# rdd0582/mri_superresolution

Hardware: AMD Instinct MI355X
Metric: 2D MRI slices/sec (train fwd+bwd) 256×256 U-Net; PSNR/SSIM vs ref (higher is better)
Workload: dtype bf16; 1 GPU; UNetSuperRes base_filters=64 depth=4, 256x256 slices -> 512x512, batch=16/GPU bf16, L1+SSIM(0.4), train step fwd+bwd+Adam+SSIM metric; global_batch=16, parallelism=dp1

## Files before the change

include/mrisr.h:

```cpp
#ifndef MRISR_H
#define MRISR_H

#include <stddef.h>
#include <stdint.h>

#ifdef __cplusplus
extern "C" {
#endif

#define MRISR_OK 0
#define MRISR_E_ARG (-1)
#define MRISR_E_SHAPE (-2)
#define MRISR_E_DTYPE (-3)
#define MRISR_E_HIP (-4)
#define MRISR_E_UNSUPPORTED (-5)

#define MRISR_F32 0
#define MRISR_BF16 1
#define MRISR_F16 2

#define MRISR_SRC_RAW 0
#define MRISR_SRC_NORM 1
#define MRISR_SRC_RELU 2
#define MRISR_SP_NONE 0
#define MRISR_SP_POOL2 1
#define MRISR_SP_UP2 2
#define MRISR_COMBINE_CONCAT 0
#define MRISR_COMBINE_BLEND 1
#ifndef MRISR_STAT_SLOTS
#define MRISR_STAT_SLOTS 16
#endif
#define MRISR_SP_HEAD 3
#define MRISR_OUT_PLAIN 0
#define MRISR_OUT_PIXEL_SHUFFLE2 1

typedef struct {
    const void* ptr;
    const float* scale;
    const float* shift;
    int32_t C, H, W;
    int32_t mode;
    int32_t spatial;
    int32_t off_y, off_x;
} mrisr_src;

typedef struct {
    int32_t dtype;
    int32_t N, H, W;
    int32_t Cin, Cout;
    int32_t ksize;
    int32_t nsrc;
    int32_t combine;
    int32_t out_mode;
    int32_t groups;
    int32_t relu_out;
    mrisr_src src[2];
    const float* blend_alpha;
    const void* wpacked;
    const float* bias;
    void* out;
    double* stats;
    const void* relu_mask;
    int32_t cu_limit;
    int32_t reserved_;
    const void* wpacked_ring;
} mrisr_conv_desc;

const char* mrisr_last_error(void);
int mrisr_version(void);
int mrisr_stat_slots(void);

size_t mrisr_packed_weight_bytes(int dtype, int Cout, int Cin, int ksize);
#define MRISR_PACK_RING 256
#define MRISR_PACK_UPADJ 512
int mrisr_conv_ring_bn(int dtype, int Cout, int Cin, int ksize);
size_t mrisr_packed_weight_bytes_ring(int dtype, int Cout, int Cin, int ksize);
int mrisr_pack_weights(int dtype, const float* w, int Cout, int Cin, int ksize, int transpose_flip,
                       void* packed, void* stream);
typedef struct {
    const float* w;
    void* packed;
    int32_t Cout, Cin, ksize, transpose_flip;
} mrisr_pack_job;
int mrisr_pack_weights_batched(int dtype, const mrisr_pack_job* jobs_device, int njobs, void* stream);
int mrisr_conv_forward(const mrisr_conv_desc* d, void* stream);
int mrisr_conv_variant(const mrisr_conv_desc* d, int wgrad, char* out, size_t n);
int mrisr_conv_wgrad(const mrisr_conv_desc* d, const void* dy, float* dw, float* workspace, size_t workspace_floats,
                     void* stream);
size_t mrisr_conv_wgrad_workspace_floats(const mrisr_conv_desc* d);

size_t mrisr_packed_weight_bytes_upadj(int dtype, int Cout, int Cin, int ksize);
int mrisr_conv_upadj(const mrisr_conv_desc* d, const void* g, void* d_low, void* stream);

int mrisr_stem_forward(int dtype, const float* x, const float* w, void* out, double* stats,
                       int N, int H, int W, int Cout, int groups, void* stream);
int mrisr_stem_wgrad(int dtype, const float* x, const void* dy, float* dw,
                     int N, int H, int W, int Cout, void* stream);
int mrisr_stem_forward_multi(int dtype, const float* x, const float* w, void* out, double* stats,
                             int N, int H, int W, int Cin, int Cout, int groups, void* stream);
int mrisr_stem_wgrad_multi(int dtype, const float* x, const void* dy, float* dw,
                           int N, int H, int W, int Cin, int Cout, void* stream);

int mrisr_gn_finalize(const double* stats, const float* gamma, const float* beta, float* scale,
                      float* shift, float* meanrstd, int N, int C, int groups, double count,
                      float eps, void* stream);

int mrisr_norm_pool2(int dtype, const void* x, const float* scale, const float* shift, void* out, int N,
                     int H, int W, int C, void* stream);
int mrisr_norm_upsample2(int dtype, const void* x, const float* scale, const float* shift, void* out, int N,
                         int h, int w, int C, void* stream);
int mrisr_norm_blend(int dtype, const void* x0, const float* scale0, const float* shift0, const void* x1,
                     const float* scale1, const float* shift1, const float* alpha, void* out, int N, int H, int W,
                     int C, void* stream);
int mrisr_upsample2_stats(int dtype, const void* z_low, void* z, double* stats, int N, int h, int w, int C,
                          int groups, void* stream);
int mrisr_upsample2_adjoint(int dtype, const void* dz, void* dz_low, int N, int h, int w, int C, void* stream);

typedef struct {
    const void* da;
    int32_t C_total;
    int32_t c_off;
    int32_t H, W;
    int32_t spatial;
    int32_t off_y, off_x;
    int32_t weight_mode;
    const float* head_out;
    const float* head_w;
    float* head_part;
    float* head_dw;
    float* head_db;
} mrisr_consumer;

int mrisr_act_bwd_reduce(int dtype, const void* x, const float* scale, const float* shift,
                         const float* meanrstd, int nconsumers, const mrisr_consumer* consumers,
                         const float* blend_alpha, void* g, float* red, float* alpha_slots, int N, int H, int W,
                         int C, int groups, void* stream);
int mrisr_act_bwd_finalize(const float* red, const float* gamma, const float* meanrstd, float* dgamma,
                           float* dbeta, float* coef, int N, int C, int groups, double count,
                           const float* alpha_slots, const float* alpha, float* dalpha, float alpha_sign, void* stream);
int mrisr_act_bwd_apply(int dtype, const void* x, const void* g, const float* coef, void* dx, int N,
                        int H, int W, int C, int out_mode, float* dbias, void* stream);
typedef struct mrisr_gn_bwd_fin {
    const float* red;
    const float* gamma;
    const float* meanrstd;
    float* dgamma;
    float* dbeta;
    const float* alpha_slots;
    const float* alpha;
    float* dalpha;
    double count;
    float alpha_sign;
    int32_t groups;
} mrisr_gn_bwd_fin;
int mrisr_act_bwd_apply_fused(int dtype, const void* x, const float* scale, const float* shift, int nconsumers,
                              const mrisr_consumer* consumers, const float* blend_alpha, const float* coef,
                              const mrisr_gn_bwd_fin* fin, void* dx, int N, int H, int W, int C, void* stream);
int mrisr_act_bwd_onepass_slots(void);
int mrisr_act_bwd_onepass_barrier_words(void);
int mrisr_act_bwd_onepass_ok(int dtype, int nconsumers, const mrisr_consumer* consumers, int N, int H, int W, int C);
int mrisr_act_bwd_onepass(int dtype, const void* x, const float* scale, const float* shift, const float* meanrstd,
                          int nconsumers, const mrisr_consumer* consumers, float* red, uint32_t* arrive,
                          const mrisr_gn_bwd_fin* fin, void* dx, int N, int H, int W, int C, void* stream);
int mrisr_act_bwd_apply_fused_unshuffle(int dtype, const void* x, const float* scale, const float* shift,
                                        const mrisr_consumer* consumer, const float* blend_alpha,
                                        const mrisr_gn_bwd_fin* fin, void* dx, float* dbias, int N, int H, int W, int C,
                                        void* stream);
typedef struct mrisr_blend_branch {
    const void* x;
    const float* scale;
    const float* shift;
    const float* meanrstd;
    float* red;
    float* alpha_slots;
    int32_t weight_mode;
    int32_t reserved_;
} mrisr_blend_branch;
int mrisr_act_bwd_blend_ok(int dtype, int N, int H, int W, int C);
int mrisr_act_bwd_blend_reduce(int dtype, const void* da, const mrisr_blend_branch* ps, const mrisr_blend_branch* bil,
                               const float* blend_alpha, int N, int H, int W, int C, int groups, void* stream);
int mrisr_act_bwd_blend_apply(int dtype, const void* da, const mrisr_blend_branch* ps, const mrisr_blend_branch* bil,
                              const float* blend_alpha, const mrisr_gn_bwd_fin* fin_ps, const mrisr_gn_bwd_fin* fin_bil,
                              void* dx_ps, void* dx_bil, float* dbias, int N, int H, int W, int C, void* stream);
int mrisr_channel_sum(int dtype, const void* x, float* out, size_t npix, int C, void* stream);

int mrisr_head_forward(int dtype, const void* x, const float* scale, const float* shift,
                       const float* w, const float* b, float* out, int N, int H, int W, int C,
                       void* stream);
int mrisr_head_backward(int dtype, const void* x, const float* scale, const float* shift,
                        const float* w, const float* out, const float* dout, void* da, float* dw,
                        float* db, int N, int H, int W, int C, void* stream);
int mrisr_head_forward_multi(int dtype, const void* x, const float* scale, const float* shift,
                             const float* w, const float* b, float* out, int N, int H, int W, int C,
                             int K, void* stream);
int mrisr_head_backward_multi(int dtype, const void* x, const float* scale, const float* shift,
                              const float* w, const float* out, const float* dout, void* da,
                              float* dw, float* db, int N, int H, int W, int C, int K, void* stream);

int mrisr_ssim_l1_forward(const float* a, const float* b, double* sums, float* coef, int N, int H,
                          int W, float val_range, float sigma, void* stream);
int mrisr_ssim_l1_backward(const float* a, const float* b, const float* coef, const double* sums,
                           const float* gscale, float l1_w, float ssim_w, float* da, int N, int H,
                           int W, float sigma, void* stream);
int mrisr_ssim_l1_forward_win(const float* a, const float* b, double* sums, float* coef, int N, int H, int W,
                              float val_range, float sigma, int window_size, void* stream);
int mrisr_ssim_l1_backward_win(const float* a, const float* b, const float* coef, const double* sums,
                               const float* gscale, float l1_w, float ssim_w, float* da, int N, int H, int W,
                               float sigma, int window_size, void* stream);

int mrisr_loss_finalize(const double* sums, int N, int H, int W, float l1_w, float ssim_w, float* out,
                        void* stream);

int mrisr_image_metrics(const float* a, const float* b, double* sums, int N, int H, int W, float val_range, float sigma,
                        int window_size, void* stream);
int mrisr_metrics_finalize(const double* sums, int N, int H, int W, float val_range, double* out, void* stream);

int mrisr_vgg_input_channels(void);
int mrisr_vgg_input_forward(int dtype, const float* x, void* out, size_t npix, void* stream);
int mrisr_vgg_input_backward(int dtype, const void* dx3, const float* gscale, float scale, float* dimg,
                             size_t npix, void* stream);
int mrisr_maxpool2_forward(int dtype, const void* x, void* out, int N, int H, int W, int C, void* stream);
int mrisr_maxpool2_backward(int dtype, const void* x, const void* dy, void* dx, int N, int H, int W, int C,
                            int relu_gate, void* stream);
int mrisr_feature_loss(int dtype, const void* a, const void* b, size_t n, int kind, double* sum16, float* out,
                       void* da, int relu_gate, void* stream);

int mrisr_adam_step(float* p, const float* g, float* m, float* v, size_t n, float lr, float beta1,
                    float beta2, float eps, float weight_decay, int step, float grad_scale,
                    void* stream);
int mrisr_adam_step_amp(float* p, const float* g, float* m, float* v, size_t n, float lr, float beta1, float beta2,
                        float eps, float weight_decay, int* step_device, float grad_mul,
                        const float* loss_scale_device, const float* found_inf_device, void* stream);

int mrisr_u8_histogram(const uint8_t* img, size_t pixels_per_image, int batch, unsigned* hist, void* stream);
int mrisr_u8_percentile_normalise(const uint8_t* img, const unsigned* hist, size_t pixels_per_image, int batch,
                                  double q_lo, double q_hi, float* out, float* lohi, void* stream);
int mrisr_f32_to_u8(const float* x, uint8_t* out, size_t n, void* stream);

#define MRISR_UP2_BILINEAR 0
#define MRISR_UP2_BICUBIC 1
#define MRISR_UP2_SHARP_BILINEAR 2
int mrisr_u8_upscale2(const uint8_t* in, uint8_t* out_u8, float* out_f32, int batch, int h, int w, int method, void* stream);
int mrisr_u8_to_unit_f32(const uint8_t* img, float* out, size_t n, void* stream);

typedef struct {
    float cos_a, sin_a;
    int32_t rotate;
    int32_t flip;
    int32_t fill;
    float brightness;
} mrisr_aug_geo;
typedef struct {
    float contrast;
    int32_t mean;
    float noise_sigma;
    uint32_t seed;
} mrisr_aug_photo;
int mrisr_augment_geo_u8(const uint8_t* in, uint8_t* out, int batch, int H, int W, const mrisr_aug_geo* params_device,
                         const double* mean_device, void* stream);
int mrisr_augment_finish_u8(const uint8_t* in, float* out, int batch, size_t pixels_per_image,
                            const mrisr_aug_photo* params_device, const double* mean_device, void* stream);

int mrisr_lowfield_dirichlet(int n, double crop_factor, float* re, float* im);
size_t mrisr_lowfield_workspace_bytes(int batch, int H, int W);
int mrisr_lowfield_simulate(const uint8_t* high, int batch, int H, int W, double crop_factor, const float* row_re,
                            const float* row_im, const float* col_re, const float* col_im, float sigma,
                            const float* noise_re, const float* noise_im, const unsigned long long* seeds_device,
                            void* workspace, uint8_t* out_u8, float* out_f32, void* stream);

int mrisr_lowfield_dirichlet_any(int n, double crop_factor, float* re, float* im);
int mrisr_lowfield_simulate_f32(const float* high, int batch, int H, int W, double crop_factor, const float* row_re,
                                const float* row_im, const float* col_re, const float* col_im, float sigma,
                                const float* noise_re, const float* noise_im, const unsigned long long* seeds_device,
                                void* workspace, float* out_f32, void* stream);

#define MRISR_WINDOW_F32 0
#define MRISR_WINDOW_I16 1
size_t mrisr_f32_percentile_workspace_bytes(int batch);
int mrisr_f32_percentile_bounds(const float* x, size_t pixels_per_image, int batch, double q_lo, double q_hi, float* lohi,
                                void* workspace, void* stream);
int mrisr_f32_window_normalise(const float* x, const float* lohi, size_t pixels_per_image, int batch, float* out, void* stream);
int mrisr_f32_window_restore(const float* y, const float* lohi, size_t pixels_per_image, int batch, int out_dtype, void* out,
                             void* stream);

#define MRISR_RESAMPLE_LINEAR 1
#define MRISR_RESAMPLE_CUBIC 2
#define MRISR_RESAMPLE_AREA 3
#define MRISR_RESAMPLE_LANCZOS4 4
int mrisr_resample_taps(int method, int src, int dst, int max_taps, int* ntaps, short* index, float* weight);
int mrisr_f32_resample_letterbox(const float* in, int batch, int H, int W, const short* y_index, const float* y_weight,
                                 int y_taps, int new_h, const short* x_index, const float* x_weight, int x_taps, int new_w,
                                 int out_h, int out_w, int y_off, int x_off, float pad_value, int clip, float* out_f32,
                                 uint8_t* out_u8, void* stream);

#define MRISR_VOLBLEND_SET 0
#define MRISR_VOLBLEND_ADD 1
#define MRISR_VOLBLEND_FINISH 2
int mrisr_f32_volume_up2_blend(const float* plane, int axis, int X, int Y, int Z, float* acc, int mode, int count, int out_dtype,
                               void* out, void* stream);

int mrisr_f32_volume_down2(const float* src, int X, int Y, int Z, int axes_mask, float* dst, void* stream);
int mrisr_f32_volume_up2(const float* src, int X, int Y, int Z, int axes_mask, int method, float* dst, void* stream);
int mrisr_f32_volume_metrics(const float* a, const float* b, int X, int Y, int Z, float val_range, float sigma, int window_size,
                             double* sums, void* stream);
int mrisr_volume_metrics_finalize(const double* sums, int X, int Y, int Z, float val_range, double* out, void* stream);
int mrisr_f32_volume_metrics_masked(const float* a, const float* b, const uint8_t* mask, int X, int Y, int Z, float val_range,
                                    float sigma, int window_size, double* sums7, void* stream);
int mrisr_volume_metrics_finalize_masked(const double* sums7, int X, int Y, int Z, float val_range, double* out11, void* stream);

size_t mrisr_f32_volume_otsu_workspace_bytes(void);
int mrisr_f32_volume_otsu_mask(const float* vol, int X, int Y, int Z, uint8_t* mask_out, double* stats, void* workspace,
                               void* stream);
#define MRISR_MORPH_DILATE 0
#define MRISR_MORPH_ERODE 1
int mrisr_u8_volume_morph(const uint8_t* src, int X, int Y, int Z, int radius, int op, uint8_t* dst, uint8_t* tmp, void* stream);

int mrisr_u8_volume_label(const uint8_t* mask, int X, int Y, int Z, int connectivity, int plane_axis, int invert, int32_t* labels,
                          void* stream);
size_t mrisr_u8_volume_label_workspace_bytes(int X, int Y, int Z);
int mrisr_u8_volume_keep_largest(const uint8_t* mask, int X, int Y, int Z, int connectivity, uint8_t* dst, double* stats3,
                                 void* workspace, void* stream);
int mrisr_u8_volume_fill_holes(const uint8_t* mask, int X, int Y, int Z, int plane_axis, uint8_t* dst, double* stats1, void* workspace,
                               void* stream);

#ifdef __cplusplus
}
#endif
#endif
```

mri_superresolution_amd/_lib.py:

```python
from __future__ import annotations

import ctypes as C
import os

from .tuning import TUNING

_HERE = os.path.dirname(os.path.abspath(__file__))
LIB_PATH = TUNING.lib_path or os.path.join(_HERE, "libmrisr.so")

F32, BF16, F16 = 0, 1, 2
SRC_RAW, SRC_NORM, SRC_RELU = 0, 1, 2
SP_NONE, SP_POOL2, SP_UP2, SP_HEAD = 0, 1, 2, 3
COMBINE_CONCAT, COMBINE_BLEND = 0, 1
OUT_PLAIN, OUT_PIXEL_SHUFFLE2 = 0, 1
UP2_BILINEAR, UP2_BICUBIC, UP2_SHARP_BILINEAR = 0, 1, 2
WINDOW_F32, WINDOW_I16 = 0, 1
VOLBLEND_SET, VOLBLEND_ADD, VOLBLEND_FINISH = 0, 1, 2
MORPH_DILATE, MORPH_ERODE = 0, 1
RESAMPLE_LINEAR, RESAMPLE_CUBIC, RESAMPLE_AREA, RESAMPLE_LANCZOS4 = 1, 2, 3, 4
PACK_RING = 256
PACK_UPADJ = 512
STAT_SLOTS = 16

_vp, _fp, _dp, _i, _f, _d, _sz = C.c_void_p, C.c_void_p, C.c_void_p, C.c_int, C.c_float, C.c_double, C.c_size_t


class Src(C.Structure):
    _fields_ = [("ptr", _vp), ("scale", _fp), ("shift", _fp), ("C", C.c_int32), ("H", C.c_int32),
                ("W", C.c_int32), ("mode", C.c_int32), ("spatial", C.c_int32), ("off_y", C.c_int32),
                ("off_x", C.c_int32)]


class ConvDesc(C.Structure):
    _fields_ = [("dtype", C.c_int32), ("N", C.c_int32), ("H", C.c_int32), ("W", C.c_int32),
                ("Cin", C.c_int32), ("Cout", C.c_int32), ("ksize", C.c_int32), ("nsrc", C.c_int32),
                ("combine", C.c_int32), ("out_mode", C.c_int32), ("groups", C.c_int32),
                ("relu_out", C.c_int32), ("src", Src * 2), ("blend_alpha", _fp), ("wpacked", _vp),
                ("bias", _fp), ("out", _vp), ("stats", _dp), ("relu_mask", _vp), ("cu_limit", C.c_int32),
                ("reserved_", C.c_int32), ("wpacked_ring", _vp)]


class PackJob(C.Structure):
    _fields_ = [("w", _fp), ("packed", _vp), ("Cout", C.c_int32), ("Cin", C.c_int32), ("ksize", C.c_int32),
                ("transpose_flip", C.c_int32)]


class AugGeo(C.Structure):
    _fields_ = [("cos_a", C.c_float), ("sin_a", C.c_float), ("rotate", C.c_int32), ("flip", C.c_int32),
                ("fill", C.c_int32), ("brightness", C.c_float)]


class AugPhoto(C.Structure):
    _fields_ = [("contrast", C.c_float), ("mean", C.c_int32), ("noise_sigma", C.c_float), ("seed", C.c_uint32)]


class GnBwdFin(C.Structure):
    _fields_ = [("red", _fp), ("gamma", _fp), ("meanrstd", _fp), ("dgamma", _fp), ("dbeta", _fp),
                ("alpha_slots", _fp), ("alpha", _fp), ("dalpha", _fp), ("count", C.c_double),
                ("alpha_sign", C.c_float), ("groups", C.c_int32)]


class BlendBranch(C.Structure):
    _fields_ = [("x", _vp), ("scale", _fp), ("shift", _fp), ("meanrstd", _fp), ("red", _fp), ("alpha_slots", _fp),
                ("weight_mode", C.c_int32), ("reserved_", C.c_int32)]


class Consumer(C.Structure):
    _fields_ = [("da", _vp), ("C_total", C.c_int32), ("c_off", C.c_int32), ("H", C.c_int32),
                ("W", C.c_int32), ("spatial", C.c_int32), ("off_y", C.c_int32), ("off_x", C.c_int32),
                ("weight_mode", C.c_int32), ("head_out", _fp), ("head_w", _fp), ("head_part", _fp),
                ("head_dw", _fp), ("head_db", _fp)]


SIGNATURES = {
    "mrisr_last_error": (C.c_char_p, []),
    "mrisr_version": (_i, []),
    "mrisr_stat_slots": (_i, []),
    "mrisr_packed_weight_bytes": (_sz, [_i, _i, _i, _i]),
    "mrisr_conv_ring_bn": (_i, [_i, _i, _i, _i]),
    "mrisr_packed_weight_bytes_ring": (_sz, [_i, _i, _i, _i]),
    "mrisr_pack_weights": (_i, [_i, _fp, _i, _i, _i, _i, _vp, _vp]),
    "mrisr_pack_weights_batched": (_i, [_i, _vp, _i, _vp]),
    "mrisr_conv_forward": (_i, [C.POINTER(ConvDesc), _vp]),
    "mrisr_packed_weight_bytes_upadj": (_sz, [_i, _i, _i, _i]),
    "mrisr_conv_upadj": (_i, [C.POINTER(ConvDesc), _vp, _vp, _vp]),
    "mrisr_conv_variant": (_i, [C.POINTER(ConvDesc), _i, C.c_char_p, _sz]),
    "mrisr_conv_wgrad": (_i, [C.POINTER(ConvDesc), _vp, _fp, _fp, _sz, _vp]),
    "mrisr_conv_wgrad_workspace_floats": (_sz, [C.POINTER(ConvDesc)]),
    "mrisr_stem_forward": (_i, [_i, _fp, _fp, _vp, _dp, _i, _i, _i, _i, _i, _vp]),
    "mrisr_stem_wgrad": (_i, [_i, _fp, _vp, _fp, _i, _i, _i, _i, _vp]),
    "mrisr_stem_forward_multi": (_i, [_i, _fp, _fp, _vp, _dp, _i, _i, _i, _i, _i, _i, _vp]),
    "mrisr_stem_wgrad_multi": (_i, [_i, _fp, _vp, _fp, _i, _i, _i, _i, _i, _vp]),
    "mrisr_gn_finalize": (_i, [_dp, _fp, _fp, _fp, _fp, _fp, _i, _i, _i, _d, _f, _vp]),
    "mrisr_norm_pool2": (_i, [_i, _vp, _fp, _fp, _vp, _i, _i, _i, _i, _vp]),
    "mrisr_norm_upsample2": (_i, [_i, _vp, _fp, _fp, _vp, _i, _i, _i, _i, _vp]),
    "mrisr_norm_blend": (_i, [_i, _vp, _fp, _fp, _vp, _fp, _fp, _fp, _vp, _i, _i, _i, _i, _vp]),
    "mrisr_upsample2_stats": (_i, [_i, _vp, _vp, _dp, _i, _i, _i, _i, _i, _vp]),
    "mrisr_upsample2_adjoint": (_i, [_i, _vp, _vp, _i, _i, _i, _i, _vp]),
    "mrisr_act_bwd_reduce": (_i, [_i, _vp, _fp, _fp, _fp, _i, C.POINTER(Consumer), _fp, _vp, _fp, _fp, _i, _i, _i, _i, _i, _vp]),
    "mrisr_act_bwd_finalize": (_i, [_fp, _fp, _fp, _fp, _fp, _fp, _i, _i, _i, _d, _fp, _fp, _fp, _f, _vp]),
    "mrisr_act_bwd_apply": (_i, [_i, _vp, _vp, _fp, _vp, _i, _i, _i, _i, _i, _fp, _vp]),
    "mrisr_act_bwd_apply_fused": (_i, [_i, _vp, _fp, _fp, _i, C.POINTER(Consumer), _fp, _fp, C.POINTER(GnBwdFin), _vp, _i, _i,
                                       _i, _i, _vp]),
    "mrisr_act_bwd_onepass_slots": (_i, []),
    "mrisr_act_bwd_onepass_barrier_words": (_i, []),
    "mrisr_act_bwd_onepass_ok": (_i, [_i, _i, C.POINTER(Consumer), _i, _i, _i, _i]),
    "mrisr_act_bwd_onepass": (_i, [_i, _vp, _fp, _fp, _fp, _i, C.POINTER(Consumer), _fp, _vp, C.POINTER(GnBwdFin), _vp, _i, _i, _i,
                                   _i, _vp]),
    "mrisr_act_bwd_apply_fused_unshuffle": (_i, [_i, _vp, _fp, _fp, C.POINTER(Consumer), _fp, C.POINTER(GnBwdFin), _vp, _fp, _i,
                                                 _i, _i, _i, _vp]),
    "mrisr_act_bwd_blend_ok": (_i, [_i, _i, _i, _i, _i]),
    "mrisr_act_bwd_blend_reduce": (_i, [_i, _vp, C.POINTER(BlendBranch), C.POINTER(BlendBranch), _fp, _i, _i, _i, _i, _i, _vp]),
    "mrisr_act_bwd_blend_apply": (_i, [_i, _vp, C.POINTER(BlendBranch), C.POINTER(BlendBranch), _fp, C.POINTER(GnBwdFin),
                                       C.POINTER(GnBwdFin), _vp, _vp, _fp, _i, _i, _i, _i, _vp]),
    "mrisr_channel_sum": (_i, [_i, _vp, _fp, _sz, _i, _vp]),
    "mrisr_head_forward": (_i, [_i, _vp, _fp, _fp, _fp, _fp, _fp, _i, _i, _i, _i, _vp]),
    "mrisr_head_backward": (_i, [_i, _vp, _fp, _fp, _fp, _fp, _fp, _vp, _fp, _fp, _i, _i, _i, _i, _vp]),
    "mrisr_head_forward_multi": (_i, [_i, _vp, _fp, _fp, _fp, _fp, _fp, _i, _i, _i, _i, _i, _vp]),
    "mrisr_head_backward_multi": (_i, [_i, _vp, _fp, _fp, _fp, _fp, _fp, _vp, _fp, _fp, _i, _i, _i, _i, _i, _vp]),
    "mrisr_ssim_l1_forward": (_i, [_fp, _fp, _dp, _fp, _i, _i, _i, _f, _f, _vp]),
    "mrisr_ssim_l1_backward": (_i, [_fp, _fp, _fp, _dp, _fp, _f, _f, _fp, _i, _i, _i, _f, _vp]),
    "mrisr_ssim_l1_forward_win": (_i, [_fp, _fp, _dp, _fp, _i, _i, _i, _f, _f, _i, _vp]),
    "mrisr_ssim_l1_backward_win": (_i, [_fp, _fp, _fp, _dp, _fp, _f, _f, _fp, _i, _i, _i, _f, _i, _vp]),
    "mrisr_loss_finalize": (_i, [_dp, _i, _i, _i, _f, _f, _fp, _vp]),
    "mrisr_image_metrics": (_i, [_fp, _fp, _dp, _i, _i, _i, _f, _f, _i, _vp]),
    "mrisr_metrics_finalize": (_i, [_dp, _i, _i, _i, _f, _dp, _vp]),
    "mrisr_vgg_input_channels": (_i, []),
    "mrisr_vgg_input_forward": (_i, [_i, _fp, _vp, _sz, _vp]),
    "mrisr_vgg_input_backward": (_i, [_i, _vp, _fp, _f, _fp, _sz, _vp]),
    "mrisr_maxpool2_forward": (_i, [_i, _vp, _vp, _i, _i, _i, _i, _vp]),
    "mrisr_maxpool2_backward": (_i, [_i, _vp, _vp, _vp, _i, _i, _i, _i, _i, _vp]),
    "mrisr_feature_loss": (_i, [_i, _vp, _vp, _sz, _i, _dp, _fp, _vp, _i, _vp]),
    "mrisr_adam_step": (_i, [_fp, _fp, _fp, _fp, _sz, _f, _f, _f, _f, _f, _i, _f, _vp]),
    "mrisr_adam_step_amp": (_i, [_fp, _fp, _fp, _fp, _sz, _f, _f, _f, _f, _f, _vp, _f, _fp, _fp, _vp]),
    "mrisr_u8_histogram": (_i, [_vp, _sz, _i, _vp, _vp]),
    "mrisr_u8_percentile_normalise": (_i, [_vp, _vp, _sz, _i, _d, _d, _fp, _fp, _vp]),
    "mrisr_f32_to_u8": (_i, [_fp, _vp, _sz, _vp]),
    "mrisr_u8_upscale2": (_i, [_vp, _vp, _fp, _i, _i, _i, _i, _vp]),
    "mrisr_u8_to_unit_f32": (_i, [_vp, _fp, _sz, _vp]),
    "mrisr_augment_geo_u8": (_i, [_vp, _vp, _i, _i, _i, _vp, _dp, _vp]),
    "mrisr_augment_finish_u8": (_i, [_vp, _fp, _i, _sz, _vp, _dp, _vp]),
    "mrisr_lowfield_dirichlet": (_i, [_i, _d, _fp, _fp]),
    "mrisr_lowfield_workspace_bytes": (_sz, [_i, _i, _i]),
    "mrisr_lowfield_simulate": (_i, [_vp, _i, _i, _i, _d, _fp, _fp, _fp, _fp, _f, _fp, _fp, _vp, _vp, _vp, _fp, _vp]),
    "mrisr_lowfield_dirichlet_any": (_i, [_i, _d, _fp, _fp]),
    "mrisr_lowfield_simulate_f32": (_i, [_fp, _i, _i, _i, _d, _fp, _fp, _fp, _fp, _f, _fp, _fp, _vp, _vp, _fp, _vp]),
    "mrisr_resample_taps": (_i, [_i, _i, _i, _i, _vp, _vp, _fp]),
    "mrisr_f32_resample_letterbox": (_i, [_fp, _i, _i, _i, _vp, _fp, _i, _i, _vp, _fp, _i, _i, _i, _i, _i, _i, _f, _i, _fp, _vp, _vp]),
    "mrisr_f32_percentile_workspace_bytes": (_sz, [_i]),
    "mrisr_f32_percentile_bounds": (_i, [_fp, _sz, _i, _d, _d, _fp, _vp, _vp]),
    "mrisr_f32_window_normalise": (_i, [_fp, _fp, _sz, _i, _fp, _vp]),
    "mrisr_f32_window_restore": (_i, [_fp, _fp, _sz, _i, _i, _vp, _vp]),
    "mrisr_f32_volume_up2_blend": (_i, [_fp, _i, _i, _i, _i, _fp, _i, _i, _i, _vp, _vp]),
    "mrisr_f32_volume_down2": (_i, [_fp, _i, _i, _i, _i, _fp, _vp]),
    "mrisr_f32_volume_up2": (_i, [_fp, _i, _i, _i, _i, _i, _fp, _vp]),
    "mrisr_f32_volume_metrics": (_i, [_fp, _fp, _i, _i, _i, _f, _f, _i, _dp, _vp]),
    "mrisr_volume_metrics_finalize": (_i, [_dp, _i, _i, _i, _f, _dp, _vp]),
    "mrisr_f32_volume_metrics_masked": (_i, [_fp, _fp, _vp, _i, _i, _i, _f, _f, _i, _dp, _vp]),
    "mrisr_volume_metrics_finalize_masked": (_i, [_dp, _i, _i, _i, _f, _dp, _vp]),
    "mrisr_f32_volume_otsu_workspace_bytes": (_sz, []),
    "mrisr_f32_volume_otsu_mask": (_i, [_fp, _i, _i, _i, _vp, _dp, _vp, _vp]),
    "mrisr_u8_volume_morph": (_i, [_vp, _i, _i, _i, _i, _i, _vp, _vp, _vp]),
    "mrisr_u8_volume_label": (_i, [_vp, _i, _i, _i, _i, _i, _i, _vp, _vp]),
    "mrisr_u8_volume_label_workspace_bytes": (_sz, [_i, _i, _i]),
    "mrisr_u8_volume_keep_largest": (_i, [_vp, _i, _i, _i, _i, _vp, _dp, _vp, _vp]),
    "mrisr_u8_volume_fill_holes": (_i, [_vp, _i, _i, _i, _i, _vp, _dp, _vp, _vp]),
}

_lib = None
ABI_VERSION = 314


def load():
    global _lib
    if _lib is not None:
        return _lib
    if not os.path.exists(LIB_PATH):
        raise RuntimeError(
            f"{LIB_PATH} not found: the HIP kernel library is not built. Run "
            "`python -m mri_superresolution_amd.build` (needs hipcc); there is no CPU fallback.")
    lib = C.CDLL(LIB_PATH)
    missing = [name for name in SIGNATURES if not hasattr(lib, name)]
    if missing:
        raise RuntimeError(f"{LIB_PATH} lacks {len(missing)} symbol(s) of include/mrisr.h ({', '.join(missing[:4])}...): "
                           "header/library drift - rebuild with `python -m mri_superresolution_amd.build`")
    for name, (res, args) in SIGNATURES.items():
        fn = getattr(lib, name)
        fn.restype = res
        fn.argtypes = args
    if int(lib.mrisr_version()) != ABI_VERSION:
        raise RuntimeError(f"{LIB_PATH} is version {int(lib.mrisr_version())}, these bindings need {ABI_VERSION} (struct layouts "
                           "changed): rebuild with `python -m mri_superresolution_amd.build`")
    global STAT_SLOTS
    STAT_SLOTS = int(lib.mrisr_stat_slots())
    _lib = lib
    return lib


def check(rc: int, what: str = ""):
    if rc != 0:
        msg = load().mrisr_last_error().decode("utf-8", "replace")
        raise RuntimeError(f"libmrisr {what} failed ({rc}): {msg}")


timer = None


def call(name: str, *args, nbytes=None):
    if timer is not None and nbytes is not None and timer.enabled:
        timer.launch(name, 0.0, lambda: check(getattr(load(), name)(*args), name), nbytes=float(nbytes))
        return
    check(getattr(load(), name)(*args), name)


def ptr(t):
    return None if t is None else t.data_ptr()


inplace_epoch = 0


def bump_inplace_epoch():
    global inplace_epoch
    inplace_epoch += 1


_NUM_CUS = None


def num_cus() -> int:
    global _NUM_CUS
    if _NUM_CUS is None:
        import torch
        _NUM_CUS = int(torch.cuda.get_device_properties(torch.cuda.current_device()).multi_processor_count)
    return _NUM_CUS


def stream_ptr():
    import torch
    return torch.cuda.current_stream().cuda_stream
```

mri_superresolution_amd/csrc/api.cpp:

```cpp
#include "common.h"
thread_local char g_mrisr_err[512] = "";
extern "C" const char* mrisr_last_error(void) { return g_mrisr_err; }
extern "C" int mrisr_version(void) { return 314; }
extern "C" int mrisr_stat_slots(void) { return MRISR_STAT_SLOTS; }
```

mri_superresolution_amd/csrc/conv_pack.hip:

```cpp
#include "conv_common.h"
#include "conv_upadj.h"

template <typename T>
__global__ void pack_weights_kernel(const float* __restrict__ w, T* __restrict__ out, int Cout, int Cin,
                                    int KS, int flip, int BN, int ncb, int nchunks) {
    constexpr int BK = kRowBytes / (int)sizeof(T);
    const int ntaps = KS * KS;
    const size_t total = (size_t)ncb * nchunks * ntaps * BN * BK;
    const int Co = flip ? Cin : Cout, Ci = flip ? Cout : Cin;
    for (size_t idx = blockIdx.x * (size_t)blockDim.x + threadIdx.x; idx < total;
         idx += (size_t)gridDim.x * blockDim.x) {
        size_t r = idx;
        const int e = r % BK; r /= BK;
        const int row = r % BN; r /= BN;
        const int tap = r % ntaps; r /= ntaps;
        const int kc = r % nchunks;
        const int cb = r / nchunks;
        constexpr int EPC = 16 / (int)sizeof(T);
        const int q = tap * BN + row;
        const int chunk_pos = e / EPC, chunk = chunk_pos ^ ((q >> 2) & 3);
        const int k = kc * BK + chunk * EPC + (e % EPC);
        const int co = cb * BN + row;
        float v = 0.f;
        if (co < Co && k < Ci) {
            if (!flip) v = w[((size_t)co * ntaps + tap) * Cin + k];
            else v = w[((size_t)k * ntaps + (ntaps - 1 - tap)) * Cin + co];
        }
        out[idx] = from_f32<T>(v);
    }
}

struct PackJobDev { const float* w; void* packed; int Cout, Cin, ksize, flip; };
template <typename T>
__global__ void pack_weights_batched_kernel(const PackJobDev* __restrict__ jobs) {
    constexpr int BK = kRowBytes / (int)sizeof(T);
    constexpr int EPC = 16 / (int)sizeof(T);
    const PackJobDev j = jobs[blockIdx.y];
    const int KS = j.ksize, ntaps = KS * KS, Cin = j.Cin, Cout = j.Cout, flip = j.flip & 1;
    const int Co = flip ? Cin : Cout, Ci = flip ? Cout : Cin;
    const float* __restrict__ w = j.w;
    auto gather = [&](int co, int tap, int k0, Vec16<T>& v) {
#pragma unroll
        for (int e = 0; e < EPC; ++e) {
            const int k = k0 + e;
            float x = 0.f;
            if (co < Co && k < Ci) x = !flip ? w[((size_t)co * ntaps + tap) * Cin + k] : w[((size_t)k * ntaps + (ntaps - 1 - tap)) * Cin + co];
            v.set(e, x);
        }
    };
    if (j.flip & MRISR_PACK_UPADJ) {
        if (!conv_upadj_image_bytes(TypeTraits<T>::kDtype, Cout, Cin, KS)) return;
        const int RS = upadj_rs(Cout), K9 = ntaps * Cout;
        const size_t nchunk = (size_t)Cin * RS / EPC;
        for (size_t idx = blockIdx.x * (size_t)blockDim.x + threadIdx.x; idx < nchunk; idx += (size_t)gridDim.x * blockDim.x) {
            const int ci = (int)(idx * EPC / RS), k0 = (int)(idx * EPC % RS);
            Vec16<T> v;
#pragma unroll
            for (int e = 0; e < EPC; ++e) {
                const int k = k0 + e;
                v.set(e, k < K9 ? w[((size_t)(k % Cout) * ntaps + k / Cout) * Cin + ci] : 0.f);
            }
            store_vec16((T*)j.packed + idx * EPC, v);
        }
        return;
    }
    if (j.flip & MRISR_PACK_RING) {
        const int RBN = conv_ring_bn(TypeTraits<T>::kDtype, Co, Ci, KS);
        if (RBN == 0) return;
        const int rnch = Ci / 16;
        const size_t nchunk = (size_t)(Co / RBN) * rnch * ntaps * RBN * 2;
        for (size_t idx = blockIdx.x * (size_t)blockDim.x + threadIdx.x; idx < nchunk; idx += (size_t)gridDim.x * blockDim.x) {
            size_t r = idx;
            const int pos = r & 1; r >>= 1;
            const int row = r % RBN; r /= RBN;
            const int tap = r % ntaps; r /= ntaps;
            const int kc = r % rnch;
            const int cb = r / rnch;
            const int slot = pos ^ ((row >> 3) & 1);
            Vec16<T> v;
            gather(cb * RBN + row, tap, kc * 16 + slot * 8, v);
            store_vec16((T*)j.packed + idx * EPC, v);
        }
        return;
    }
    const int BN = Co >= 64 ? 64 : 32;
    const int ncb = (Co + BN - 1) / BN, nchunks = (Ci + BK - 1) / BK;
    const size_t nchunk = (size_t)ncb * nchunks * ntaps * BN * 4;
    for (size_t idx = blockIdx.x * (size_t)blockDim.x + threadIdx.x; idx < nchunk; idx += (size_t)gridDim.x * blockDim.x) {
        size_t r = idx;
        const int pos = r & 3; r >>= 2;
        const int row = r % BN; r /= BN;
        const int tap = r % ntaps; r /= ntaps;
        const int kc = r % nchunks;
        const int cb = r / nchunks;
        const int q = tap * BN + row;
        const int chunk = pos ^ ((q >> 2) & 3);
        Vec16<T> v;
        gather(cb * BN + row, tap, kc * BK + chunk * EPC, v);
        store_vec16((T*)j.packed + idx * EPC, v);
    }
}

extern "C" int mrisr_pack_weights_batched(int dtype, const mrisr_pack_job* jobs_device, int njobs, void* stream) {
    static_assert(sizeof(PackJobDev) == sizeof(mrisr_pack_job), "mrisr_pack_job layout");
    if (!jobs_device || njobs <= 0 || njobs > 65535) MRISR_FAIL(MRISR_E_ARG, "pack_weights_batched: bad job table");
    dim3 grid(256, njobs);
    if (dtype == MRISR_BF16)
        pack_weights_batched_kernel<bf16_t><<<grid, 256, 0, (hipStream_t)stream>>>((const PackJobDev*)jobs_device);
    else if (dtype == MRISR_F16)
        pack_weights_batched_kernel<f16_t><<<grid, 256, 0, (hipStream_t)stream>>>((const PackJobDev*)jobs_device);
    else if (dtype == MRISR_F32)
        pack_weights_batched_kernel<float><<<grid, 256, 0, (hipStream_t)stream>>>((const PackJobDev*)jobs_device);
    else
        MRISR_FAIL(MRISR_E_DTYPE, "pack_weights_batched: dtype %d", dtype);
    MRISR_CHECK_LAUNCH("pack_weights_batched");
    return MRISR_OK;
}

extern "C" size_t mrisr_packed_weight_bytes(int dtype, int Cout, int Cin, int ksize) {
    const int BN = conv_choose_bn(Cout), BK = conv_bk(dtype);
    const size_t ncb = ceil_div(Cout, BN), nch = ceil_div(Cin, BK);
    return ncb * nch * (size_t)(ksize * ksize) * BN * kRowBytes;
}

extern "C" int mrisr_pack_weights(int dtype, const float* w, int Cout, int Cin, int ksize, int transpose_flip,
                                  void* packed, void* stream) {
    if (!w || !packed) MRISR_FAIL(MRISR_E_ARG, "pack_weights: null pointer");
    if (ksize != 1 && ksize != 3) MRISR_FAIL(MRISR_E_UNSUPPORTED, "pack_weights: ksize %d", ksize);
    if (transpose_flip & (MRISR_PACK_RING | MRISR_PACK_UPADJ)) {
        const int flip = transpose_flip & 1;
        if ((transpose_flip & MRISR_PACK_UPADJ) && !conv_upadj_image_bytes(dtype, Cout, Cin, ksize))
            MRISR_FAIL(MRISR_E_UNSUPPORTED, "pack_weights: no upadj layout for %d -> %d k%d dtype %d", Cin, Cout, ksize, dtype);
        if (!(transpose_flip & MRISR_PACK_UPADJ) && !mrisr_conv_ring_bn(dtype, flip ? Cin : Cout, flip ? Cout : Cin, ksize))
            MRISR_FAIL(MRISR_E_UNSUPPORTED, "pack_weights: no ring layout for %d -> %d k%d dtype %d", Cin, Cout, ksize, dtype);
        const PackJobDev job{w, packed, Cout, Cin, ksize, transpose_flip};
        PackJobDev* dj = nullptr;
        if (hipMalloc(&dj, sizeof(job)) != hipSuccess) MRISR_FAIL(MRISR_E_HIP, "pack_weights: hipMalloc");
        (void)hipMemcpyAsync(dj, &job, sizeof(job), hipMemcpyHostToDevice, (hipStream_t)stream);
        const int rc = mrisr_pack_weights_batched(dtype, (const mrisr_pack_job*)dj, 1, stream);
        (void)hipStreamSynchronize((hipStream_t)stream);
        (void)hipFree(dj);
        return rc;
    }
    transpose_flip &= 1;
    const int Co = transpose_flip ? Cin : Cout, Ci = transpose_flip ? Cout : Cin;
    const int BN = conv_choose_bn(Co), BK = conv_bk(dtype);
    const int ncb = ceil_div(Co, BN), nch = ceil_div(Ci, BK);
    const size_t total = (size_t)ncb * nch * ksize * ksize * BN * BK;
    const int blocks = (int)((total + 255) / 256 < 4096 ? (total + 255) / 256 : 4096);
    if (dtype == MRISR_BF16)
        pack_weights_kernel<bf16_t><<<blocks, 256, 0, (hipStream_t)stream>>>(w, (bf16_t*)packed, Cout, Cin, ksize,
                                                                            transpose_flip, BN, ncb, nch);
    else if (dtype == MRISR_F16)
        pack_weights_kernel<f16_t><<<blocks, 256, 0, (hipStream_t)stream>>>(w, (f16_t*)packed, Cout, Cin, ksize,
                                                                           transpose_flip, BN, ncb, nch);
    else if (dtype == MRISR_F32)
        pack_weights_kernel<float><<<blocks, 256, 0, (hipStream_t)stream>>>(w, (float*)packed, Cout, Cin, ksize,
                                                                           transpose_flip, BN, ncb, nch);
    else
        MRISR_FAIL(MRISR_E_DTYPE, "pack_weights: dtype %d", dtype);
    MRISR_CHECK_LAUNCH("pack_weights");
    return MRISR_OK;
}
```

mri_superresolution_amd/csrc/optim.hip:

```cpp
#include "common.h"

__global__ __launch_bounds__(256) void adam_kernel(float* __restrict__ p, const float* __restrict__ g,
                                                   float* __restrict__ m, float* __restrict__ v, size_t n, float lr,
                                                   float b1, float b2, float eps, float wd, float bc1, float rsqrt_bc2,
                                                   float gscale) {
    const size_t stride = (size_t)gridDim.x * blockDim.x * 4;
    for (size_t i = ((size_t)blockIdx.x * blockDim.x + threadIdx.x) * 4; i < n; i += stride) {
        if (i + 3 < n) {
            f32x4 pv = *reinterpret_cast<f32x4*>(p + i);
            const f32x4 gv = *reinterpret_cast<const f32x4*>(g + i);
            f32x4 mv = *reinterpret_cast<f32x4*>(m + i), vv = *reinterpret_cast<f32x4*>(v + i);
#pragma unroll
            for (int e = 0; e < 4; ++e) {
                const float gg = gv[e] * gscale + wd * pv[e];
                mv[e] = b1 * mv[e] + (1.f - b1) * gg;
                vv[e] = b2 * vv[e] + (1.f - b2) * gg * gg;
                pv[e] -= (lr / bc1) * mv[e] / (sqrtf(vv[e]) * rsqrt_bc2 + eps);
            }
            *reinterpret_cast<f32x4*>(p + i) = pv;
            *reinterpret_cast<f32x4*>(m + i) = mv;
            *reinterpret_cast<f32x4*>(v + i) = vv;
        } else {
            for (size_t j = i; j < n; ++j) {
                const float gg = g[j] * gscale + wd * p[j];
                m[j] = b1 * m[j] + (1.f - b1) * gg;
                v[j] = b2 * v[j] + (1.f - b2) * gg * gg;
                p[j] -= (lr / bc1) * m[j] / (sqrtf(v[j]) * rsqrt_bc2 + eps);
            }
        }
    }
}

extern "C" int mrisr_adam_step(float* p, const float* g, float* m, float* v, size_t n, float lr, float beta1,
                               float beta2, float eps, float weight_decay, int step, float grad_scale, void* stream) {
    if (!p || !g || !m || !v) MRISR_FAIL(MRISR_E_ARG, "adam_step: null pointer");
    if (step < 1) MRISR_FAIL(MRISR_E_ARG, "adam_step: step %d < 1", step);
    if (((uintptr_t)p | (uintptr_t)g | (uintptr_t)m | (uintptr_t)v) & 15) MRISR_FAIL(MRISR_E_ARG, "adam_step: buffers must be 16-byte aligned");
    const double bc1 = 1.0 - pow((double)beta1, step), bc2 = 1.0 - pow((double)beta2, step);
    const size_t nv = (n + 3) / 4;
    const int blocks = (int)((nv + 255) / 256 < 2048 ? (nv + 255) / 256 : 2048);
    adam_kernel<<<blocks ? blocks : 1, 256, 0, (hipStream_t)stream>>>(p, g, m, v, n, lr, beta1, beta2, eps, weight_decay,
                                                                     (float)bc1, (float)(1.0 / sqrt(bc2)), grad_scale);
    MRISR_CHECK_LAUNCH("adam_step");
    return MRISR_OK;
}

__global__ __launch_bounds__(256) void adam_amp_kernel(float* __restrict__ p, const float* __restrict__ g,
                                                       float* __restrict__ m, float* __restrict__ v, size_t n, float lr,
                                                       float b1, float b2, float eps, float wd, float gmul,
                                                       const int* __restrict__ step, const float* __restrict__ loss_scale,
                                                       const float* __restrict__ found_inf) {
    if (found_inf && found_inf[0] != 0.f) return;
    const float t = (float)(step[0] + 1);
    const float bc1 = 1.f - powf(b1, t), rsqrt_bc2 = rsqrtf(1.f - powf(b2, t));
    const float gscale = gmul / (loss_scale ? loss_scale[0] : 1.f);
    const size_t stride = (size_t)gridDim.x * blockDim.x * 4;
    for (size_t i = ((size_t)blockIdx.x * blockDim.x + threadIdx.x) * 4; i < n; i += stride) {
        const size_t e1 = i + 4 < n ? i + 4 : n;
        for (size_t j = i; j < e1; ++j) {
            const float gg = g[j] * gscale + wd * p[j];
            const float mj = b1 * m[j] + (1.f - b1) * gg, vj = b2 * v[j] + (1.f - b2) * gg * gg;
            m[j] = mj;
            v[j] = vj;
            p[j] -= (lr / bc1) * mj / (sqrtf(vj) * rsqrt_bc2 + eps);
        }
    }
}
__global__ void adam_amp_advance_kernel(int* step, const float* found_inf) {
    if (!(found_inf && found_inf[0] != 0.f)) step[0] += 1;
}

extern "C" int mrisr_adam_step_amp(float* p, const float* g, float* m, float* v, size_t n, float lr, float beta1,
                                   float beta2, float eps, float weight_decay, int* step_device, float grad_mul,
                                   const float* loss_scale_device, const float* found_inf_device, void* stream) {
    if (!p || !g || !m || !v || !step_device) MRISR_FAIL(MRISR_E_ARG, "adam_step_amp: null pointer");
    if (((uintptr_t)p | (uintptr_t)g | (uintptr_t)m | (uintptr_t)v) & 15) MRISR_FAIL(MRISR_E_ARG, "adam_step_amp: buffers must be 16-byte aligned");
    const size_t nv = (n + 3) / 4;
    const int blocks = (int)((nv + 255) / 256 < 2048 ? (nv + 255) / 256 : 2048);
    adam_amp_kernel<<<blocks ? blocks : 1, 256, 0, (hipStream_t)stream>>>(p, g, m, v, n, lr, beta1, beta2, eps, weight_decay,
                                                                         grad_mul, step_device, loss_scale_device, found_inf_device);
    MRISR_CHECK_LAUNCH("adam_step_amp");
    adam_amp_advance_kernel<<<1, 1, 0, (hipStream_t)stream>>>(step_device, found_inf_device);
    MRISR_CHECK_LAUNCH("adam_step_amp(advance)");
    return MRISR_OK;
}
```

mri_superresolution_amd/engine.py:

```python
from __future__ import annotations

import ctypes as C
from dataclasses import dataclass
from typing import Dict, List, Optional, Tuple

import torch

from . import _lib as L
from .launch import GN_GROUPS, Consumer, dgrad_desc, gn_finalize, marshal_consumers
from .tuning import TUNING


def _dt(dtype: torch.dtype) -> int:
    if dtype == torch.bfloat16:
        return L.BF16
    if dtype == torch.float16:
        return L.F16
    if dtype == torch.float32:
        return L.F32
    raise ValueError(f"unsupported compute dtype {dtype} (use torch.float32, torch.float16 or torch.bfloat16)")


@dataclass(frozen=True, eq=False)
class Node:
    name: str
    C: int
    gamma: str
    beta: str
    shuffled: bool = False


@dataclass(frozen=True, eq=False)
class Source:
    node: Node
    spatial: int = L.SP_NONE


@dataclass(frozen=True, eq=False)
class Layer:
    name: str
    cin: int
    cout: int
    ks: int
    srcs: Tuple[Source, ...]
    out: Node
    combine: int = L.COMBINE_CONCAT
    bias: bool = False
    out_mode: int = L.OUT_PLAIN
    pool_src: bool = False
    up_src: bool = False
    blend_src: bool = False
    post_up: bool = False


class _NodeState:
    __slots__ = ("H", "W", "raw", "stats", "scale", "shift", "meanrstd", "consumers")

    def __init__(self, stats: torch.Tensor):
        self.stats = stats
        self.H = self.W = self.raw = self.scale = self.shift = self.meanrstd = None
        self.consumers: List[Consumer] = []


class _LayerState:
    __slots__ = ("H", "W", "offs", "aux")

    def __init__(self, H: int, W: int, offs: list, aux: Optional[torch.Tensor]):
        self.H, self.W, self.offs, self.aux = H, W, offs, aux


class _Pass:
    __slots__ = ("x", "out", "dtype", "N", "arena", "nodes", "layers")

    def __getitem__(self, key):
        if key != "nodes" or self.nodes is None:
            raise KeyError(key)
        return {n.name: (self.N, s.H, s.W, s.raw, s.scale, s.shift, s.meanrstd) for n, s in self.nodes.items()}


class KernelTimer:

    def __init__(self):
        self.records = []
        self.enabled = True

    def launch(self, name: str, flops: float, fn, nbytes: float = 0.0):
        if not self.enabled:
            return fn()
        a, b = torch.cuda.Event(enable_timing=True), torch.cuda.Event(enable_timing=True)
        a.record()
        fn()
        b.record()
        self.records.append((name, flops, nbytes, a, b))

    def __enter__(self):
        L.timer = self
        return self

    def __exit__(self, *exc):
        L.timer = None

    def summary(self):
        agg = {}
        for name, flops, nbytes, a, b in self.records:
            e = agg.setdefault(name, [0, 0.0, 0.0, 0.0])
            e[0] += 1
            e[1] += flops
            e[2] += a.elapsed_time(b)
            e[3] += nbytes
        return {k: {"launches": n, "flops_per_launch": fl / n, "bytes_per_launch": by / n, "ms_per_launch": ms / n,
                    "total_ms": ms, "tflops": fl / (ms * 1e-3) / 1e12 if ms > 0 else 0.0,
                    "tbps": by / (ms * 1e-3) / 1e12 if ms > 0 else 0.0}
                for k, (n, fl, ms, by) in agg.items()}


class UNetEngine:

    def __init__(self, base_filters: int, in_channels: int = 1, out_channels: int = 1, depth: int = 4):
        if not (1 <= in_channels <= 4 and 1 <= out_channels <= 4):
            raise NotImplementedError("the HIP stem / head kernels take 1..4 image channels (in_channels, out_channels)")
        self.cin, self.cout = in_channels, out_channels
        if base_filters % 16:
            raise ValueError("base_filters must be a multiple of 16 (GroupNorm(8, base_filters // 2))")
        f = self.f = base_filters
        self.nodes: Dict[str, Node] = {}
        self.layers: List[Layer] = []

        def node(name, c, gn_prefix_w, gn_prefix_b, shuffled=False):
            n = Node(name, c, gn_prefix_w, gn_prefix_b, shuffled)
            self.nodes[name] = n
            return n

        def dconv(prefix, src: Tuple[Source, ...], cin, cout, combine=L.COMBINE_CONCAT, pool_src=False):
            a = node(f"{prefix}.double_conv.0", cout, f"{prefix}.double_conv.1.weight", f"{prefix}.double_conv.1.bias")
            self.layers.append(Layer(f"{prefix}.double_conv.0", cin, cout, 3, src, a, combine, pool_src=pool_src))
            b = node(f"{prefix}.double_conv.3", cout, f"{prefix}.double_conv.4.weight", f"{prefix}.double_conv.4.bias")
            self.layers.append(Layer(f"{prefix}.double_conv.3", cout, cout, 3, (Source(a),), b))
            return b

        self.stem = node("inc.double_conv.0", f, "inc.double_conv.1.weight", "inc.double_conv.1.bias")
        x1 = node("inc.double_conv.3", f, "inc.double_conv.4.weight", "inc.double_conv.4.bias")
        self.layers.append(Layer("inc.double_conv.3", f, f, 3, (Source(self.stem),), x1))
        if depth < 2:
            raise ValueError("depth must be >= 2")
        self.depth = depth
        xs = [x1]
        for k in range(1, depth):
            xs.append(dconv(f"down{k}.maxpool_conv.1", (Source(xs[-1]),), f * 2 ** (k - 1), f * 2 ** k, pool_src=True))
        u = xs[-1]
        for j in range(1, depth):
            skip, cout = xs[depth - 1 - j], f * 2 ** (depth - 1 - j)
            up = node(f"up{j}.up.1", cout, f"up{j}.up.2.weight", f"up{j}.up.2.bias")
            self.layers.append(Layer(f"up{j}.up.1", 2 * cout, cout, 1, (Source(u),), up, post_up=True))
            u = dconv(f"up{j}.conv", (Source(skip), Source(up)), 2 * cout, cout)
        fb = node("final_up_bilinear.1", f // 2, "final_up_bilinear.2.weight", "final_up_bilinear.2.bias")
        self.layers.append(Layer("final_up_bilinear.1", f, f // 2, 3, (Source(u),), fb, up_src=True))
        ps = node("final_up_pixelshuffle.conv", f // 2, "final_up_pixelshuffle.norm.weight",
                  "final_up_pixelshuffle.norm.bias", shuffled=True)
        self.layers.append(Layer("final_up_pixelshuffle.conv", f, 2 * f, 3, (Source(u),), ps, bias=True,
                                 out_mode=L.OUT_PIXEL_SHUFFLE2))
        fc = node("final_conv.0", f // 2, "final_conv.1.weight", "final_conv.1.bias")
        self.layers.append(Layer("final_conv.0", f // 2, f // 2, 3, (Source(fb), Source(ps)), fc,
                                 combine=L.COMBINE_BLEND, blend_src=True))
        self.head_in = fc
        self._blend_sibling: Dict[Node, Node] = {}
        for layer in self.layers:
            if layer.combine == L.COMBINE_BLEND:
                a, b = (src.node for src in layer.srcs)
                self._blend_sibling[a], self._blend_sibling[b] = b, a
        self._packed: Dict[tuple, torch.Tensor] = {}
        self._packed_token = None
        self.timer: Optional[KernelTimer] = None

    def _launch(self, kind, desc, fn):
        if self.timer is None:
            return fn()
        flops = 2.0 * desc.N * desc.H * desc.W * desc.Cin * desc.Cout * desc.ksize * desc.ksize
        if kind == "upadj":
            flops /= 4
        buf = C.create_string_buffer(96)
        L.call("mrisr_conv_variant", C.byref(desc), {"wgrad": 1, "upadj": 2}.get(kind, 0), buf, 96)
        self.timer.launch(buf.value.decode(), flops, fn)

    def _packed_buf(self, layer: Layer, w, dt: int, flip: int, ring: bool = False, upadj: bool = False):
        key = (layer.name, dt, "upadj") if upadj else (layer.name, dt, flip, "ring") if ring else (layer.name, dt, flip)
        buf = self._packed.get(key)
        if buf is None or buf.device != w.device:
            if upadj:
                nbytes = L.load().mrisr_packed_weight_bytes_upadj(dt, layer.cout, layer.cin, layer.ks)
            else:
                size = L.load().mrisr_packed_weight_bytes_ring if ring else L.load().mrisr_packed_weight_bytes
                nbytes = size(dt, layer.cin if flip else layer.cout, layer.cout if flip else layer.cin, layer.ks)
            buf = torch.empty(nbytes, dtype=torch.uint8, device=w.device)
            self._packed[key] = buf
        return buf

    def invalidate_packed(self):
        self._packed.clear()
        self._jobs_key = None
        self._packed_token = None

    def _pack_all(self, params, dt: int, stream, token=None):
        dev = params[self.layers[0].name + ".weight"].device
        key = (dt, str(dev), tuple(params[l.name + ".weight"].data_ptr() for l in self.layers))
        if getattr(self, "_jobs_key", None) != key:
            jobs = (L.PackJob * (4 * len(self.layers) + 1))()
            i = 0
            for layer in self.layers:
                w = params[layer.name + ".weight"]
                for flip in (0, 1):
                    buf = self._packed_buf(layer, w, dt, flip)
                    j = jobs[i]
                    j.w, j.packed, j.Cout, j.Cin, j.ksize, j.transpose_flip = w.data_ptr(), buf.data_ptr(), layer.cout, layer.cin, layer.ks, flip
                    i += 1
                    co, ci = (layer.cin, layer.cout) if flip else (layer.cout, layer.cin)
                    if L.load().mrisr_conv_ring_bn(dt, co, ci, layer.ks) > 0:
                        buf = self._packed_buf(layer, w, dt, flip, ring=True)
                        j = jobs[i]
                        j.w, j.packed, j.Cout, j.Cin, j.ksize, j.transpose_flip = (w.data_ptr(), buf.data_ptr(), layer.cout, layer.cin,
                                                                                   layer.ks, flip | L.PACK_RING)
                        i += 1
                if layer.up_src and L.load().mrisr_packed_weight_bytes_upadj(dt, layer.cout, layer.cin, layer.ks) > 0:
                    buf = self._packed_buf(layer, w, dt, 0, upadj=True)
                    j = jobs[i]
                    j.w, j.packed, j.Cout, j.Cin, j.ksize, j.transpose_flip = (w.data_ptr(), buf.data_ptr(), layer.cout, layer.cin,
                                                                               layer.ks, L.PACK_UPADJ)
                    i += 1
            self._jobs_bytes = sum(4 * params[l.name + ".weight"].numel() for l in self.layers) * 2 + \
                sum(b.numel() for k, b in self._packed.items() if k[1] == dt)
            host = torch.frombuffer(bytearray(bytes(jobs)), dtype=torch.uint8)
            self._jobs_dev = host.to(dev)
            self._jobs_n = i
            self._jobs_key = key
        L.call("mrisr_pack_weights_batched", dt, self._jobs_dev.data_ptr(), self._jobs_n, stream, nbytes=self._jobs_bytes)
        self._packed_token = (dt, token)

    def _desc(self, layer: Layer, p: _Pass, dt: int, params, fused_blend: bool = False) -> L.ConvDesc:
        g = p.layers[layer]
        d = L.ConvDesc()
        d.dtype, d.N, d.H, d.W = dt, p.N, g.H, g.W
        d.Cin, d.Cout, d.ksize, d.nsrc = layer.cin, layer.cout, layer.ks, len(layer.srcs)
        d.combine, d.out_mode, d.groups, d.relu_out = layer.combine, layer.out_mode, GN_GROUPS, 0
        d.cu_limit = TUNING.cu_limit
        if layer.blend_src and not fused_blend:
            d.nsrc, d.combine = 1, L.COMBINE_CONCAT
            d.src[0].ptr = g.aux.data_ptr()
            d.src[0].C, d.src[0].H, d.src[0].W = layer.cin, g.H, g.W
            d.src[0].mode, d.src[0].spatial = L.SRC_RAW, L.SP_NONE
            return d
        for i, (s, (oy, ox)) in enumerate(zip(layer.srcs, g.offs)):
            n = p.nodes[s.node]
            if layer.pool_src or layer.up_src:
                d.src[i].ptr = g.aux.data_ptr()
                d.src[i].C, d.src[i].H, d.src[i].W = s.node.C, g.H, g.W
                d.src[i].mode, d.src[i].spatial = L.SRC_RAW, L.SP_NONE
                continue
            d.src[i].ptr = n.raw.data_ptr()
            d.src[i].scale = n.scale.data_ptr()
            d.src[i].shift = n.shift.data_ptr()
            d.src[i].C, d.src[i].H, d.src[i].W = s.node.C, n.H, n.W
            d.src[i].mode, d.src[i].spatial = L.SRC_NORM, s.spatial
            d.src[i].off_y, d.src[i].off_x = oy, ox
        if layer.combine == L.COMBINE_BLEND:
            d.blend_alpha = params["alpha"].data_ptr()
        return d

    @staticmethod
    def _virtual_hw(s: Source, n: _NodeState):
        if s.spatial == L.SP_POOL2:
            return n.H // 2, n.W // 2
        if s.spatial == L.SP_UP2:
            return 2 * n.H, 2 * n.W
        return n.H, n.W

    def forward(self, params, x: torch.Tensor, dtype: torch.dtype, training: bool, weights_token=None):
        dt = _dt(dtype)
        dev = x.device
        N, _, H, W = x.shape
        es = 4 if dtype == torch.float32 else 2
        mins = 2 ** (self.depth - 1)
        if H < mins or W < mins:
            raise ValueError(f"input must be at least {mins}x{mins} ({self.depth - 1} 2x2 max-pools)")
        st = L.stream_ptr()
        f = self.f
        p = _Pass()
        p.x, p.dtype, p.N = x, dtype, N
        per = L.STAT_SLOTS * N * GN_GROUPS * 2
        p.arena = torch.zeros(len(self.nodes) * per, dtype=torch.float64, device=dev)
        ns = p.nodes = {n: _NodeState(p.arena[i * per:(i + 1) * per]) for i, n in enumerate(self.nodes.values())}
        p.layers = {}

        def finalize(n: Node):
            o = ns[n]
            o.scale, o.shift, o.meanrstd = gn_finalize(o.stats, params[n.gamma], params[n.beta], N, n.C, o.H, o.W, st)

        if training or weights_token is None or self._packed_token != (dt, weights_token):
            self._pack_all(params, dt, st, weights_token)
        s = ns[self.stem]
        s.H, s.W = H, W
        s.raw = torch.empty((N, H, W, f), dtype=dtype, device=dev)
        L.call("mrisr_stem_forward_multi", dt, x.data_ptr(), params["inc.double_conv.0.weight"].data_ptr(),
               s.raw.data_ptr(), s.stats.data_ptr(), N, H, W, self.cin, f, GN_GROUPS, st,
               nbytes=N * H * W * (4 * self.cin + f * es))
        finalize(self.stem)

        for layer in self.layers:
            sn = ns[layer.srcs[0].node]
            sC = layer.srcs[0].node.C
            vh, vw = self._virtual_hw(layer.srcs[0], sn)
            aux = None
            if layer.pool_src:
                vh, vw = sn.H // 2, sn.W // 2
                aux = torch.empty((N, vh, vw, sC), dtype=dtype, device=dev)
                L.call("mrisr_norm_pool2", dt, sn.raw.data_ptr(), sn.scale.data_ptr(), sn.shift.data_ptr(),
                       aux.data_ptr(), N, sn.H, sn.W, sC, st, nbytes=N * sn.H * sn.W * sC * es * 1.25)
            if layer.up_src:
                vh, vw = 2 * sn.H, 2 * sn.W
                aux = torch.empty((N, vh, vw, sC), dtype=dtype, device=dev)
                L.call("mrisr_norm_upsample2", dt, sn.raw.data_ptr(), sn.scale.data_ptr(), sn.shift.data_ptr(),
                       aux.data_ptr(), N, sn.H, sn.W, sC, st, nbytes=N * sn.H * sn.W * sC * es * 5)
            fused_blend = (layer.blend_src and not training and es == 2 and layer.cout == 32
                           and (layer.name, dt, 0, "ring") in self._packed)
            if layer.blend_src and not fused_blend:
                a, b = sn, ns[layer.srcs[1].node]
                if (a.H, a.W, sC) != (b.H, b.W, layer.srcs[1].node.C):
                    raise RuntimeError(f"{layer.name}: blend sources differ in shape")
                aux = torch.empty((N, a.H, a.W, sC), dtype=dtype, device=dev)
                L.call("mrisr_norm_blend", dt, a.raw.data_ptr(), a.scale.data_ptr(), a.shift.data_ptr(), b.raw.data_ptr(),
                       b.scale.data_ptr(), b.shift.data_ptr(), params["alpha"].data_ptr(), aux.data_ptr(),
                       N, a.H, a.W, sC, st, nbytes=N * a.H * a.W * sC * es * 3)
            offs = []
            for src in layer.srcs:
                h, w = (vh, vw) if (layer.pool_src or layer.up_src) else self._virtual_hw(src, ns[src.node])
                dy, dx = vh - h, vw - w
                if dy < 0 or dx < 0:
                    raise RuntimeError(f"{layer.name}: source larger than the conv input")
                offs.append((dy // 2, dx // 2))
            p.layers[layer] = _LayerState(vh, vw, offs, aux)
            o, oC = ns[layer.out], layer.out.C
            if layer.out_mode == L.OUT_PIXEL_SHUFFLE2 or layer.post_up:
                o.H, o.W = 2 * vh, 2 * vw
            else:
                o.H, o.W = vh, vw
            o.raw = torch.empty((N, o.H, o.W, oC), dtype=dtype, device=dev)
            d = self._desc(layer, p, dt, params, fused_blend)
            d.wpacked = self._packed[(layer.name, dt, 0)].data_ptr()
            d.wpacked_ring = L.ptr(self._packed.get((layer.name, dt, 0, "ring")))
            d.bias = params[layer.name + ".bias"].data_ptr() if layer.bias else None
            if layer.post_up:
                zlow = torch.empty((N, vh, vw, oC), dtype=dtype, device=dev)
                d.out, d.stats = zlow.data_ptr(), None
            else:
                d.out, d.stats = o.raw.data_ptr(), o.stats.data_ptr()
            self._launch("fwd", d, lambda: L.call("mrisr_conv_forward", C.byref(d), st))
            if layer.post_up:
                L.call("mrisr_upsample2_stats", dt, zlow.data_ptr(), o.raw.data_ptr(), o.stats.data_ptr(),
                       N, vh, vw, oC, GN_GROUPS, st, nbytes=N * vh * vw * oC * es * 5)
            finalize(layer.out)

        hn, hC = ns[self.head_in], self.head_in.C
        p.out = torch.empty((N, self.cout, hn.H, hn.W), dtype=torch.float32, device=dev)
        L.call("mrisr_head_forward_multi", dt, hn.raw.data_ptr(), hn.scale.data_ptr(), hn.shift.data_ptr(),
               params["final_conv.3.weight"].data_ptr(), params["final_conv.3.bias"].data_ptr(), p.out.data_ptr(),
               N, hn.H, hn.W, hC, self.cout, st, nbytes=N * hn.H * hn.W * (hC * es + 4 * self.cout))
        return p.out, (p if training else None)

    def backward(self, params, grads, ctx: _Pass, dout: torch.Tensor, bucket_hook=None):
        dtype = ctx.dtype
        dt = _dt(dtype)
        es = 4 if dtype == torch.float32 else 2
        N = ctx.N
        x = ctx.x
        dev = x.device
        st = L.stream_ptr()
        ns, ls = ctx.nodes, ctx.layers
        dout = dout.contiguous()

        narr = N * L.load().mrisr_act_bwd_onepass_barrier_words()
        SL = L.load().mrisr_act_bwd_onepass_slots() if es == 2 else 1
        red_sizes = [SL * N * n.C * 2 + 256 + narr + (N * (n.C + 1) if n is self.head_in else 0) for n in self.nodes.values()]
        red_arena = torch.zeros(sum(red_sizes), dtype=torch.float32, device=dev)
        red_off = {}
        o = 0
        for n, sz in zip(self.nodes.values(), red_sizes):
            red_off[n] = (o, sz)
            o += sz

        blend_dx: Dict[Node, torch.Tensor] = {}

        def node_backward(n: Node, dbias=None) -> torch.Tensor:
            if n in blend_dx:
                return blend_dx.pop(n)
            s = ns[n]
            H, W, Cn = s.H, s.W, n.C
            consumers = s.consumers
            s.consumers = []
            cons = marshal_consumers(consumers)
            ncons = len(consumers)
            c0 = consumers[0]
            own = all((c.H, c.W, c.off_y, c.off_x) == (H, W, 0, 0) for c in consumers if c.spatial == L.SP_NONE)
            plain = all(c.spatial in (L.SP_NONE, L.SP_HEAD) for c in consumers)
            window = (not plain and H % 2 == 0 and W % 2 == 0 and own
                      and sum(c.spatial == L.SP_POOL2 for c in consumers) == 1
                      and all(c.spatial in (L.SP_POOL2, L.SP_NONE) for c in consumers))
            fused = (not n.shuffled) and (plain or window)
            fused_ps = n.shuffled and ncons == 1 and c0.spatial == L.SP_NONE and H % 2 == 0 and W % 2 == 0 and own
            uses_alpha = any(c.weight_mode != 0 for c in consumers)
            alpha_ptr = params["alpha"].data_ptr() if uses_alpha else None
            red = red_arena[red_off[n][0]:red_off[n][0] + red_off[n][1]]
            blend_branch = c0.weight_mode != 0 and c0.spatial == L.SP_NONE
            slots = red[SL * N * Cn * 2:] if blend_branch else None
            alpha_sign = 1.0 if c0.weight_mode == 1 else -1.0
            nx = N * H * W * Cn * es
            nda = sum(N * c.H * c.W * (8 if c.spatial == L.SP_HEAD else Cn * es) for c in consumers)
            count = float((Cn // GN_GROUPS) * H * W)
            dalpha_ptr = grads["alpha"].data_ptr() if slots is not None else None
            gn = (red.data_ptr(), params[n.gamma].data_ptr(), s.meanrstd.data_ptr(), grads[n.gamma].data_ptr(),
                  grads[n.beta].data_ptr())

            def onepass():
                arrive = red[SL * N * Cn * 2 + 256:SL * N * Cn * 2 + 256 + narr]
                f = L.GnBwdFin(*gn, None, None, None, count, 1.0, GN_GROUPS)
                dx = torch.empty_like(s.raw)
                L.call("mrisr_act_bwd_onepass", dt, s.raw.data_ptr(), s.scale.data_ptr(), s.shift.data_ptr(),
                       s.meanrstd.data_ptr(), ncons, cons, red.data_ptr(), arrive.data_ptr(), C.byref(f),
                       dx.data_ptr(), N, H, W, Cn, st, nbytes=2 * nx + nda)
                return dx

            def reduce(g):
                L.call("mrisr_act_bwd_reduce", dt, s.raw.data_ptr(), s.scale.data_ptr(), s.shift.data_ptr(),
                       s.meanrstd.data_ptr(), ncons, cons, alpha_ptr, L.ptr(g), red.data_ptr(), L.ptr(slots),
                       N, H, W, Cn, GN_GROUPS, st, nbytes=nx + nda + (nx if g is not None else 0))

            def fused_unshuffle():
                f = L.GnBwdFin(*gn, L.ptr(slots), alpha_ptr, dalpha_ptr, count, alpha_sign, GN_GROUPS)
                dx = torch.empty((N, H // 2, W // 2, 4 * Cn), dtype=dtype, device=dev)
                L.call("mrisr_act_bwd_apply_fused_unshuffle", dt, s.raw.data_ptr(), s.scale.data_ptr(),
                       s.shift.data_ptr(), cons, alpha_ptr, C.byref(f), dx.data_ptr(), L.ptr(dbias), N, H, W, Cn, st,
                       nbytes=2 * nx + nda)
                return dx

            def fused_apply():
                f = L.GnBwdFin(*gn, L.ptr(slots), alpha_ptr, dalpha_ptr, count, alpha_sign, GN_GROUPS)
                dx = torch.empty_like(s.raw)
                L.call("mrisr_act_bwd_apply_fused", dt, s.raw.data_ptr(), s.scale.data_ptr(), s.shift.data_ptr(),
                       ncons, cons, alpha_ptr, None, C.byref(f), dx.data_ptr(), N, H, W, Cn, st,
                       nbytes=2 * nx + nda)
                return dx

            def general(g):
                coef = torch.empty(3 * N * Cn, dtype=torch.float32, device=dev)
                L.call("mrisr_act_bwd_finalize", *gn, coef.data_ptr(), N, Cn, GN_GROUPS, count, L.ptr(slots), alpha_ptr, dalpha_ptr,
                       alpha_sign, st)
                if n.shuffled:
                    dx = torch.empty((N, H // 2, W // 2, 4 * Cn), dtype=dtype, device=dev)
                    mode = L.OUT_PIXEL_SHUFFLE2
                else:
                    dx = torch.empty_like(s.raw)
                    mode = L.OUT_PLAIN
                L.call("mrisr_act_bwd_apply", dt, s.raw.data_ptr(), g.data_ptr(), coef.data_ptr(), dx.data_ptr(),
                       N, H, W, Cn, mode, L.ptr(dbias) if n.shuffled else None, st, nbytes=3 * nx)
                return dx

            def blend_pair():
                sib = self._blend_sibling.get(n)
                if sib is None or not (fused_ps and blend_branch) or sib.shuffled or sib.C != Cn or (c0.C_total, c0.c_off) != (Cn, 0):
                    return None
                t = ns[sib]
                if len(t.consumers) != 1 or (t.H, t.W) != (H, W):
                    return None
                k = t.consumers[0]
                if (k.da is not c0.da or k.weight_mode not in (1, 2) or k.weight_mode == c0.weight_mode or k.spatial != L.SP_NONE
                        or (k.H, k.W, k.off_y, k.off_x, k.C_total, k.c_off) != (H, W, 0, 0, Cn, 0)):
                    return None
                if not L.load().mrisr_act_bwd_blend_ok(dt, N, H, W, Cn):
                    return None
                t.consumers = []
                red_s = red_arena[red_off[sib][0]:red_off[sib][0] + red_off[sib][1]]
                slots_s = red_s[SL * N * Cn * 2:]
                bp = L.BlendBranch(s.raw.data_ptr(), s.scale.data_ptr(), s.shift.data_ptr(), s.meanrstd.data_ptr(), red.data_ptr(),
                                   slots.data_ptr(), c0.weight_mode, 0)
                bb = L.BlendBranch(t.raw.data_ptr(), t.scale.data_ptr(), t.shift.data_ptr(), t.meanrstd.data_ptr(), red_s.data_ptr(),
                                   slots_s.data_ptr(), k.weight_mode, 0)
                L.call("mrisr_act_bwd_blend_reduce", dt, c0.da.data_ptr(), C.byref(bp), C.byref(bb), alpha_ptr, N, H, W, Cn,
                       GN_GROUPS, st, nbytes=3 * nx)
                fp = L.GnBwdFin(*gn, slots.data_ptr(), alpha_ptr, dalpha_ptr, count, alpha_sign, GN_GROUPS)
                fb = L.GnBwdFin(red_s.data_ptr(), params[sib.gamma].data_ptr(), t.meanrstd.data_ptr(), grads[sib.gamma].data_ptr(),
                                grads[sib.beta].data_ptr(), slots_s.data_ptr(), alpha_ptr, dalpha_ptr, count,
                                1.0 if k.weight_mode == 1 else -1.0, GN_GROUPS)
                dx = torch.empty((N, H // 2, W // 2, 4 * Cn), dtype=dtype, device=dev)
                dx_sib = torch.empty_like(t.raw)
                L.call("mrisr_act_bwd_blend_apply", dt, c0.da.data_ptr(), C.byref(bp), C.byref(bb), alpha_ptr, C.byref(fp),
                       C.byref(fb), dx.data_ptr(), dx_sib.data_ptr(), L.ptr(dbias), N, H, W, Cn, st, nbytes=5 * nx)
                blend_dx[sib] = dx_sib
                return dx

            dx = blend_pair()
            if dx is not None:
                return dx
            op_blocks = -(-(H * W) // ((256 // max(Cn // 8, 1)) * 8)) if Cn >= 8 else 1 << 30
            if (fused and slots is None and not uses_alpha
                    and op_blocks <= (128 if bucket_hook is not None else 256)
                    and L.load().mrisr_act_bwd_onepass_ok(dt, ncons, cons, N, H, W, Cn)):
                return onepass()
            g = None if (fused or fused_ps) else torch.empty_like(s.raw)
            reduce(g)
            if fused_ps:
                return fused_unshuffle()
            if fused:
                return fused_apply()
            return general(g)

        hn, hC = ns[self.head_in], self.head_in.C
        ho = red_off[self.head_in][0] + SL * N * hC * 2 + 256 + narr
        if self.cout == 1:
            hn.consumers.append(Consumer(dout, hC, 0, hn.H, hn.W, L.SP_HEAD, 0, 0, head=(
                ctx.out, params["final_conv.3.weight"], red_arena[ho:ho + N * (hC + 1)], grads["final_conv.3.weight"],
                grads["final_conv.3.bias"])))
        else:
            dah = torch.empty_like(hn.raw)
            L.call("mrisr_head_backward_multi", dt, hn.raw.data_ptr(), hn.scale.data_ptr(), hn.shift.data_ptr(),
                   params["final_conv.3.weight"].data_ptr(), ctx.out.data_ptr(), dout.data_ptr(), dah.data_ptr(),
                   grads["final_conv.3.weight"].data_ptr(), grads["final_conv.3.bias"].data_ptr(), N, hn.H, hn.W, hC,
                   self.cout, st, nbytes=N * hn.H * hn.W * (2 * hC * es + 8 * self.cout))
            hn.consumers.append(Consumer(dah, hC, 0, hn.H, hn.W, L.SP_NONE, 0, 0))

        side = None
        main = torch.cuda.current_stream()
        side_default = L.num_cus() * 13 // 32 if self.f <= 64 else L.num_cus() * 3 // 8
        side_cus = side_default if TUNING.wgrad_cus < 0 else TUNING.wgrad_cus
        if TUNING.wgrad_stream and self.timer is None:
            side = getattr(self, "_side_stream", None)
            if side is None or side.device != dev:
                side = self._side_stream = torch.cuda.Stream(device=dev, priority=-1)
        main_cus = max(8, L.num_cus() - side_cus) if side is not None and side_cus > 0 else TUNING.cu_limit
        user_hook = bucket_hook
        if bucket_hook is not None and side is not None:
            def bucket_hook(name):
                ev2 = torch.cuda.Event()
                ev2.record(main)
                side.wait_event(ev2)
                with torch.cuda.stream(side):
                    user_hook(name)
        for layer in reversed(self.layers):
            geo = ls[layer]
            fuse_bias = layer.bias and layer.out.shuffled
            dy = node_backward(layer.out, grads[layer.name + ".bias"] if fuse_bias else None)
            if layer.out is self.head_in and bucket_hook:
                bucket_hook("final_conv.3")
            if layer.post_up:
                dyl = torch.empty((N, geo.H, geo.W, layer.cout), dtype=dtype, device=dev)
                L.call("mrisr_upsample2_adjoint", dt, dy.data_ptr(), dyl.data_ptr(), N, geo.H, geo.W, layer.cout, st,
                       nbytes=N * geo.H * geo.W * layer.cout * es * 5)
                dy = dyl
            d = self._desc(layer, ctx, dt, params)
            need = L.load().mrisr_conv_wgrad_workspace_floats(C.byref(d))
            ws = getattr(self, "_wgrad_ws", None)
            if ws is None or ws.numel() < need or ws.device != dev:
                ws = self._wgrad_ws = torch.empty(max(need, 1), dtype=torch.float32, device=dev)
            if side is None:
                self._launch("wgrad", d, lambda: L.call("mrisr_conv_wgrad", C.byref(d), dy.data_ptr(),
                                                        grads[layer.name + ".weight"].data_ptr(), ws.data_ptr(),
                                                        ws.numel(), st))
            else:
                ev = torch.cuda.Event()
                ev.record(main)
                side.wait_event(ev)
                d.cu_limit = side_cus
                L.call("mrisr_conv_wgrad", C.byref(d), dy.data_ptr(), grads[layer.name + ".weight"].data_ptr(),
                       ws.data_ptr(), ws.numel(), side.cuda_stream)
                dy.record_stream(side)
            if layer.bias and not fuse_bias:
                L.call("mrisr_channel_sum", dt, dy.data_ptr(), grads[layer.name + ".bias"].data_ptr(),
                       N * geo.H * geo.W, layer.cout, st, nbytes=N * geo.H * geo.W * layer.cout * es)
            src0 = layer.srcs[0].node
            upk = self._packed.get((layer.name, dt, "upadj")) if layer.up_src else None
            if upk is not None:
                sn = ns[src0]
                ud = L.ConvDesc()
                ud.dtype, ud.N, ud.H, ud.W = dt, N, geo.H, geo.W
                ud.Cin, ud.Cout, ud.ksize, ud.nsrc = layer.cin, layer.cout, layer.ks, 1
                ud.wpacked = upk.data_ptr()
                ud.cu_limit = main_cus
                dlow = torch.empty((N, sn.H, sn.W, layer.cin), dtype=dtype, device=dev)
                self._launch("upadj", ud, lambda: L.call("mrisr_conv_upadj", C.byref(ud), dy.data_ptr(), dlow.data_ptr(), st))
                sn.consumers.append(Consumer(dlow, layer.cin, 0, sn.H, sn.W, L.SP_NONE, 0, 0))
                if bucket_hook:
                    bucket_hook(layer.name)
                continue
            dain = torch.empty((N, geo.H, geo.W, layer.cin), dtype=dtype, device=dev)
            dd = dgrad_desc(dt, dy, layer.cin, layer.cout, layer.ks, self._packed[(layer.name, dt, 1)], dain,
                            self._packed.get((layer.name, dt, 1, "ring")), main_cus)
            self._launch("dgrad", dd, lambda: L.call("mrisr_conv_forward", C.byref(dd), st))
            if layer.combine == L.COMBINE_BLEND:
                for src, wm in zip(layer.srcs, (1, 2)):
                    ns[src.node].consumers.append(Consumer(dain, layer.cin, 0, geo.H, geo.W, L.SP_NONE, 0, 0, weight_mode=wm))
            elif layer.up_src:
                sn = ns[src0]
                dlow = torch.empty((N, sn.H, sn.W, layer.cin), dtype=dtype, device=dev)
                L.call("mrisr_upsample2_adjoint", dt, dain.data_ptr(), dlow.data_ptr(), N, sn.H, sn.W, layer.cin, st,
                       nbytes=N * sn.H * sn.W * layer.cin * es * 5)
                sn.consumers.append(Consumer(dlow, layer.cin, 0, sn.H, sn.W, L.SP_NONE, 0, 0))
            else:
                coff = 0
                for src, (oy, ox) in zip(layer.srcs, geo.offs):
                    sp = L.SP_POOL2 if layer.pool_src else src.spatial
                    ns[src.node].consumers.append(Consumer(dain, layer.cin, coff, geo.H, geo.W, sp, oy, ox))
                    coff += src.node.C
            if bucket_hook:
                bucket_hook(layer.name)

        dy = node_backward(self.stem)
        sH, sW = ns[self.stem].H, ns[self.stem].W
        L.call("mrisr_stem_wgrad_multi", dt, x.data_ptr(), dy.data_ptr(), grads["inc.double_conv.0.weight"].data_ptr(),
               N, sH, sW, self.cin, self.f, st, nbytes=N * sH * sW * self.cin * (4 + self.f * es))
        if bucket_hook:
            bucket_hook("inc.double_conv.0")
        if side is not None:
            main.wait_stream(side)
        ctx.nodes = ctx.layers = ctx.arena = None
```

mri_superresolution_amd/optim.py:

```python
from __future__ import annotations

import torch

from . import _lib as L


class FusedAdam(torch.optim.Optimizer):
    _step_supports_amp_scaling = True

    def __init__(self, model, lr=1e-3, betas=(0.9, 0.999), eps=1e-8, weight_decay=0.0, device_step=False):
        if not hasattr(model, "flat_params"):
            raise TypeError("FusedAdam needs a model with flat parameter storage (UNetSuperRes)")
        self.model = model
        super().__init__(list(model.parameters()), dict(lr=lr, betas=betas, eps=eps, weight_decay=weight_decay))
        self._step = 0
        self._step_dev = None
        self.device_step = bool(device_step)
        self.dp_grad_scale = 1.0
        self._alloc()

    def _alloc(self):
        flat = self.model.flat_params
        self.exp_avg = torch.zeros_like(flat)
        self.exp_avg_sq = torch.zeros_like(flat)
        self._flat_ptr = flat.data_ptr()

    @torch.no_grad()
    def step(self, closure=None):
        loss = closure() if closure is not None else None
        m = self.model
        if m.flat_params.data_ptr() != self._flat_ptr:
            raise RuntimeError("model storage was re-created (model.to(...) after the optimizer was built)")
        if not m.flat_params.is_cuda:
            raise RuntimeError("FusedAdam runs on the GPU only (no CPU fallback)")
        plist = getattr(self, "_plist", None)
        if plist is None or self._plist_ptr != self._flat_ptr:
            plist = self._plist = [(p, m._grad_views[name]) for name, p in m.named_parameters()]
            self._plist_ptr = self._flat_ptr
        for p, gv in plist:
            if p.grad is not None and p.grad.data_ptr() != gv.data_ptr():
                gv.copy_(p.grad)
        g = self.param_groups[0]
        loss_scale, found_inf = getattr(self, "grad_scale", None), getattr(self, "found_inf", None)
        if loss_scale is not None or found_inf is not None or self._step_dev is not None or self.device_step:
            if self._step_dev is None:
                self._step_dev = torch.tensor([self._step], dtype=torch.int32, device=m.flat_params.device)
            ls = None if loss_scale is None else loss_scale.detach().to(torch.float32).reshape(-1)
            fi = None if found_inf is None else found_inf.detach().to(torch.float32).reshape(-1)
            L.call("mrisr_adam_step_amp", m.flat_params.data_ptr(), m.flat_grads.data_ptr(), self.exp_avg.data_ptr(),
                   self.exp_avg_sq.data_ptr(), m.flat_params.numel(), float(g["lr"]), float(g["betas"][0]),
                   float(g["betas"][1]), float(g["eps"]), float(g["weight_decay"]), self._step_dev.data_ptr(),
                   float(self.dp_grad_scale), L.ptr(ls), L.ptr(fi), L.stream_ptr(), nbytes=28 * m.flat_params.numel())
        else:
            self._step += 1
            L.call("mrisr_adam_step", m.flat_params.data_ptr(), m.flat_grads.data_ptr(), self.exp_avg.data_ptr(),
                   self.exp_avg_sq.data_ptr(), m.flat_params.numel(), float(g["lr"]), float(g["betas"][0]),
                   float(g["betas"][1]), float(g["eps"]), float(g["weight_decay"]), self._step, float(self.dp_grad_scale),
                   L.stream_ptr(), nbytes=28 * m.flat_params.numel())
        m.mark_weights_changed()
        return loss

    def _views(self, flat):
        out = []
        for name, p in self.model.named_parameters():
            off, n = self.model._offsets[name]
            v = flat[off:off + n]
            if p.dim() == 4:
                co, ci, kh, kw = p.shape
                v = v.view(co, kh, kw, ci).permute(0, 3, 1, 2)
            else:
                v = v.view(p.shape)
            out.append(v)
        return out

    @property
    def step_count(self) -> int:
        return int(self._step_dev.item()) if self._step_dev is not None else self._step

    def set_step_count(self, step: int):
        self._step = int(step)
        if self._step_dev is not None:
            self._step_dev.fill_(int(step))

    def state_dict(self):
        groups = [{k: v for k, v in g.items() if k != "params"} for g in self.param_groups]
        n = len(self.param_groups[0]["params"])
        groups[0]["params"] = list(range(n))
        state = {}
        step = self.step_count
        if step > 0:
            for i, (ea, es) in enumerate(zip(self._views(self.exp_avg), self._views(self.exp_avg_sq))):
                state[i] = {"step": torch.tensor(float(step)), "exp_avg": ea.clone(), "exp_avg_sq": es.clone()}
        return {"state": state, "param_groups": groups}

    def load_state_dict(self, sd):
        for g, src in zip(self.param_groups, sd["param_groups"]):
            for k, v in src.items():
                if k != "params":
                    g[k] = v
        st = sd.get("state", {})
        if st:
            for i, (ea, es) in enumerate(zip(self._views(self.exp_avg), self._views(self.exp_avg_sq))):
                ent = st.get(i, st.get(str(i)))
                if ent is None:
                    continue
                ea.copy_(ent["exp_avg"])
                es.copy_(ent["exp_avg_sq"])
                self.set_step_count(int(float(ent["step"])))
```

Measured before the change: 2187 slices/s.

## Fuse Adam update with bf16 packed-weight image generation

```diff
diff --git a/include/mrisr.h b/include/mrisr.h
--- a/include/mrisr.h
+++ b/include/mrisr.h
@@ -231,6 +231,21 @@
 int mrisr_adam_step_amp(float* p, const float* g, float* m, float* v, size_t n, float lr, float beta1, float beta2,
                         float eps, float weight_decay, int* step_device, float grad_mul,
                         const float* loss_scale_device, const float* found_inf_device, void* stream);
+typedef struct {
+    int64_t off;
+    int32_t n, job0, njobs, tile0, ntiles, reserved_;
+} mrisr_adam_pack_seg;
+int mrisr_adam_pack_tiles(int Cout, int Cin, int ksize);
+int mrisr_adam_pack_flat_tile(void);
+int mrisr_adam_pack_step(int dtype, float* p, const float* g, float* m, float* v, size_t n, float lr, float beta1,
+                         float beta2, float eps, float weight_decay, int step, float grad_scale,
+                         const mrisr_pack_job* jobs_device, const mrisr_adam_pack_seg* segs_device, int nsegs,
+                         int ntiles, void* stream);
+int mrisr_adam_pack_step_amp(int dtype, float* p, const float* g, float* m, float* v, size_t n, float lr, float beta1,
+                             float beta2, float eps, float weight_decay, int* step_device, float grad_mul,
+                             const float* loss_scale_device, const float* found_inf_device,
+                             const mrisr_pack_job* jobs_device, const mrisr_adam_pack_seg* segs_device, int nsegs,
+                             int ntiles, void* stream);
 
 int mrisr_u8_histogram(const uint8_t* img, size_t pixels_per_image, int batch, unsigned* hist, void* stream);
 int mrisr_u8_percentile_normalise(const uint8_t* img, const unsigned* hist, size_t pixels_per_image, int batch,
diff --git a/mri_superresolution_amd/_lib.py b/mri_superresolution_amd/_lib.py
--- a/mri_superresolution_amd/_lib.py
+++ b/mri_superresolution_amd/_lib.py
@@ -43,6 +43,11 @@
 class PackJob(C.Structure):
     _fields_ = [("w", _fp), ("packed", _vp), ("Cout", C.c_int32), ("Cin", C.c_int32), ("ksize", C.c_int32),
                 ("transpose_flip", C.c_int32)]
+
+
+class AdamPackSeg(C.Structure):
+    _fields_ = [("off", C.c_int64), ("n", C.c_int32), ("job0", C.c_int32), ("njobs", C.c_int32), ("tile0", C.c_int32),
+                ("ntiles", C.c_int32), ("reserved_", C.c_int32)]
 
 
 class AugGeo(C.Structure):
@@ -133,6 +138,10 @@
     "mrisr_feature_loss": (_i, [_i, _vp, _vp, _sz, _i, _dp, _fp, _vp, _i, _vp]),
     "mrisr_adam_step": (_i, [_fp, _fp, _fp, _fp, _sz, _f, _f, _f, _f, _f, _i, _f, _vp]),
     "mrisr_adam_step_amp": (_i, [_fp, _fp, _fp, _fp, _sz, _f, _f, _f, _f, _f, _vp, _f, _fp, _fp, _vp]),
+    "mrisr_adam_pack_tiles": (_i, [_i, _i, _i]),
+    "mrisr_adam_pack_flat_tile": (_i, []),
+    "mrisr_adam_pack_step": (_i, [_i, _fp, _fp, _fp, _fp, _sz, _f, _f, _f, _f, _f, _i, _f, _vp, _vp, _i, _i, _vp]),
+    "mrisr_adam_pack_step_amp": (_i, [_i, _fp, _fp, _fp, _fp, _sz, _f, _f, _f, _f, _f, _vp, _f, _fp, _fp, _vp, _vp, _i, _i, _vp]),
     "mrisr_u8_histogram": (_i, [_vp, _sz, _i, _vp, _vp]),
     "mrisr_u8_percentile_normalise": (_i, [_vp, _vp, _sz, _i, _d, _d, _fp, _fp, _vp]),
     "mrisr_f32_to_u8": (_i, [_fp, _vp, _sz, _vp]),
@@ -168,7 +177,7 @@
 }
 
 _lib = None
-ABI_VERSION = 314
+ABI_VERSION = 315
 
 
 def load():
diff --git a/mri_superresolution_amd/csrc/api.cpp b/mri_superresolution_amd/csrc/api.cpp
--- a/mri_superresolution_amd/csrc/api.cpp
+++ b/mri_superresolution_amd/csrc/api.cpp
@@ -1,5 +1,5 @@
 #include "common.h"
 thread_local char g_mrisr_err[512] = "";
 extern "C" const char* mrisr_last_error(void) { return g_mrisr_err; }
-extern "C" int mrisr_version(void) { return 314; }
+extern "C" int mrisr_version(void) { return 315; }
 extern "C" int mrisr_stat_slots(void) { return MRISR_STAT_SLOTS; }
diff --git a/mri_superresolution_amd/csrc/conv_pack.h b/mri_superresolution_amd/csrc/conv_pack.h
--- /dev/null
+++ b/mri_superresolution_amd/csrc/conv_pack.h
@@ -0,0 +1,81 @@
+#pragma once
+#include "conv_common.h"
+#include "conv_upadj.h"
+
+struct PackJobDev { const float* w; void* packed; int Cout, Cin, ksize, flip; };
+
+__host__ __device__ __forceinline__ void pack_master_coord(int flip, int ntaps, int co, int tap, int k, int& mco, int& mtap, int& mci) {
+    mco = flip ? k : co;
+    mtap = flip ? ntaps - 1 - tap : tap;
+    mci = flip ? co : k;
+}
+__host__ __device__ __forceinline__ void pack_image_coord(int flip, int ntaps, int mco, int mtap, int mci, int& co, int& tap, int& k) {
+    co = flip ? mci : mco;
+    tap = flip ? ntaps - 1 - mtap : mtap;
+    k = flip ? mco : mci;
+}
+
+template <typename T> struct PackPlain {
+    static constexpr int BK = kRowBytes / (int)sizeof(T), EPC = 16 / (int)sizeof(T);
+    int BN, ncb, nchunks, ntaps;
+    __host__ __device__ PackPlain(int Co, int Ci, int ntaps_) : BN(Co >= 64 ? 64 : 32), ntaps(ntaps_) {
+        ncb = (Co + BN - 1) / BN;
+        nchunks = (Ci + BK - 1) / BK;
+    }
+    __host__ __device__ int rows() const { return ncb * BN; }
+    __host__ __device__ int chans() const { return nchunks * BK; }
+    __host__ __device__ size_t chunks() const { return (size_t)ncb * nchunks * ntaps * BN * 4; }
+    __host__ __device__ void decode(size_t idx, int& co, int& tap, int& k0) const {
+        size_t r = idx;
+        const int pos = r & 3; r >>= 2;
+        const int row = r % BN; r /= BN;
+        tap = r % ntaps; r /= ntaps;
+        const int kc = r % nchunks;
+        const int cb = r / nchunks;
+        const int q = tap * BN + row;
+        co = cb * BN + row;
+        k0 = kc * BK + (pos ^ ((q >> 2) & 3)) * EPC;
+    }
+    __host__ __device__ size_t encode(int co, int tap, int k0) const {
+        const int cb = co / BN, row = co % BN, kc = k0 / BK, chunk = (k0 % BK) / EPC;
+        const int q = tap * BN + row;
+        return ((((size_t)cb * nchunks + kc) * ntaps + tap) * BN + row) * 4 + (chunk ^ ((q >> 2) & 3));
+    }
+};
+
+struct PackRing {
+    int RBN, rnch, ntaps, ncb;
+    __host__ __device__ PackRing(int dtype, int Co, int Ci, int ksize) : RBN(conv_ring_bn(dtype, Co, Ci, ksize)), rnch(Ci / 16), ntaps(ksize * ksize) {
+        ncb = RBN ? Co / RBN : 0;
+    }
+    __host__ __device__ int rows() const { return ncb * RBN; }
+    __host__ __device__ int chans() const { return rnch * 16; }
+    __host__ __device__ size_t chunks() const { return (size_t)ncb * rnch * ntaps * RBN * 2; }
+    __host__ __device__ void decode(size_t idx, int& co, int& tap, int& k0) const {
+        size_t r = idx;
+        const int pos = r & 1; r >>= 1;
+        const int row = r % RBN; r /= RBN;
+        tap = r % ntaps; r /= ntaps;
+        const int kc = r % rnch;
+        const int cb = r / rnch;
+        co = cb * RBN + row;
+        k0 = kc * 16 + (pos ^ ((row >> 3) & 1)) * 8;
+    }
+    __host__ __device__ size_t encode(int co, int tap, int k0) const {
+        const int cb = co / RBN, row = co % RBN, kc = k0 / 16, slot = (k0 % 16) / 8;
+        return ((((size_t)cb * rnch + kc) * ntaps + tap) * RBN + row) * 2 + (slot ^ ((row >> 3) & 1));
+    }
+};
+
+struct PackUpadj {
+    int Cout, RS, K9;
+    __host__ __device__ PackUpadj(int Cout_, int ntaps) : Cout(Cout_), RS(upadj_rs(Cout_)), K9(ntaps * Cout_) {}
+    __host__ __device__ size_t chunks(int Cin, int EPC) const { return (size_t)Cin * RS / EPC; }
+    __host__ __device__ void decode(size_t idx, int EPC, int& ci, int& k0) const {
+        ci = (int)(idx * EPC / RS);
+        k0 = (int)(idx * EPC % RS);
+    }
+    __host__ __device__ void master(int k, int& mco, int& mtap) const { mco = k % Cout; mtap = k / Cout; }
+    __host__ __device__ size_t encode(int ci, int k0, int EPC) const { return ((size_t)ci * RS + k0) / EPC; }
+    __host__ __device__ int row_of(int mco, int mtap) const { return mtap * Cout + mco; }
+};
diff --git a/mri_superresolution_amd/csrc/conv_pack.hip b/mri_superresolution_amd/csrc/conv_pack.hip
--- a/mri_superresolution_amd/csrc/conv_pack.hip
+++ b/mri_superresolution_amd/csrc/conv_pack.hip
@@ -1,5 +1,4 @@
-#include "conv_common.h"
-#include "conv_upadj.h"
+#include "conv_pack.h"
 
 template <typename T>
 __global__ void pack_weights_kernel(const float* __restrict__ w, T* __restrict__ out, int Cout, int Cin,
@@ -30,10 +29,8 @@
     }
 }
 
-struct PackJobDev { const float* w; void* packed; int Cout, Cin, ksize, flip; };
 template <typename T>
 __global__ void pack_weights_batched_kernel(const PackJobDev* __restrict__ jobs) {
-    constexpr int BK = kRowBytes / (int)sizeof(T);
     constexpr int EPC = 16 / (int)sizeof(T);
     const PackJobDev j = jobs[blockIdx.y];
     const int KS = j.ksize, ntaps = KS * KS, Cin = j.Cin, Cout = j.Cout, flip = j.flip & 1;
@@ -44,59 +41,57 @@
         for (int e = 0; e < EPC; ++e) {
             const int k = k0 + e;
             float x = 0.f;
-            if (co < Co && k < Ci) x = !flip ? w[((size_t)co * ntaps + tap) * Cin + k] : w[((size_t)k * ntaps + (ntaps - 1 - tap)) * Cin + co];
+            if (co < Co && k < Ci) {
+                int mco, mtap, mci;
+                pack_master_coord(flip, ntaps, co, tap, k, mco, mtap, mci);
+                x = w[((size_t)mco * ntaps + mtap) * Cin + mci];
+            }
             v.set(e, x);
         }
     };
     if (j.flip & MRISR_PACK_UPADJ) {
         if (!conv_upadj_image_bytes(TypeTraits<T>::kDtype, Cout, Cin, KS)) return;
-        const int RS = upadj_rs(Cout), K9 = ntaps * Cout;
-        const size_t nchunk = (size_t)Cin * RS / EPC;
+        const PackUpadj L(Cout, ntaps);
+        const size_t nchunk = L.chunks(Cin, EPC);
         for (size_t idx = blockIdx.x * (size_t)blockDim.x + threadIdx.x; idx < nchunk; idx += (size_t)gridDim.x * blockDim.x) {
-            const int ci = (int)(idx * EPC / RS), k0 = (int)(idx * EPC % RS);
+            int ci, k0;
+            L.decode(idx, EPC, ci, k0);
             Vec16<T> v;
 #pragma unroll
             for (int e = 0; e < EPC; ++e) {
                 const int k = k0 + e;
-                v.set(e, k < K9 ? w[((size_t)(k % Cout) * ntaps + k / Cout) * Cin + ci] : 0.f);
+                float x = 0.f;
+                if (k < L.K9) {
+                    int mco, mtap;
+                    L.master(k, mco, mtap);
+                    x = w[((size_t)mco * ntaps + mtap) * Cin + ci];
+                }
+                v.set(e, x);
             }
             store_vec16((T*)j.packed + idx * EPC, v);
         }
         return;
     }
     if (j.flip & MRISR_PACK_RING) {
-        const int RBN = conv_ring_bn(TypeTraits<T>::kDtype, Co, Ci, KS);
-        if (RBN == 0) return;
-        const int rnch = Ci / 16;
-        const size_t nchunk = (size_t)(Co / RBN) * rnch * ntaps * RBN * 2;
+        const PackRing L(TypeTraits<T>::kDtype, Co, Ci, KS);
+        if (L.RBN == 0) return;
+        const size_t nchunk = L.chunks();
         for (size_t idx = blockIdx.x * (size_t)blockDim.x + threadIdx.x; idx < nchunk; idx += (size_t)gridDim.x * blockDim.x) {
-            size_t r = idx;
-            const int pos = r & 1; r >>= 1;
-            const int row = r % RBN; r /= RBN;
-            const int tap = r % ntaps; r /= ntaps;
-            const int kc = r % rnch;
-            const int cb = r / rnch;
-            const int slot = pos ^ ((row >> 3) & 1);
+            int co, tap, k0;
+            L.decode(idx, co, tap, k0);
             Vec16<T> v;
-            gather(cb * RBN + row, tap, kc * 16 + slot * 8, v);
+            gather(co, tap, k0, v);
             store_vec16((T*)j.packed + idx * EPC, v);
         }
         return;
     }
-    const int BN = Co >= 64 ? 64 : 32;
-    const int ncb = (Co + BN - 1) / BN, nchunks = (Ci + BK - 1) / BK;
-    const size_t nchunk = (size_t)ncb * nchunks * ntaps * BN * 4;
+    const PackPlain<T> L(Co, Ci, ntaps);
+    const size_t nchunk = L.chunks();
     for (size_t idx = blockIdx.x * (size_t)blockDim.x + threadIdx.x; idx < nchunk; idx += (size_t)gridDim.x * blockDim.x) {
-        size_t r = idx;
-        const int pos = r & 3; r >>= 2;
-        const int row = r % BN; r /= BN;
-        const int tap = r % ntaps; r /= ntaps;
-        const int kc = r % nchunks;
-        const int cb = r / nchunks;
-        const int q = tap * BN + row;
-        const int chunk = pos ^ ((q >> 2) & 3);
+        int co, tap, k0;
+        L.decode(idx, co, tap, k0);
         Vec16<T> v;
-        gather(cb * BN + row, tap, kc * BK + chunk * EPC, v);
+        gather(co, tap, k0, v);
         store_vec16((T*)j.packed + idx * EPC, v);
     }
 }
diff --git a/mri_superresolution_amd/csrc/optim.hip b/mri_superresolution_amd/csrc/optim.hip
--- a/mri_superresolution_amd/csrc/optim.hip
+++ b/mri_superresolution_amd/csrc/optim.hip
@@ -1,32 +1,56 @@
-#include "common.h"
+#include "conv_pack.h"
+
+struct AdamCoef { float step_size, b1, b2, eps, wd, rsqrt_bc2, gscale; };
+template <bool AMP>
+__device__ __forceinline__ void adam_update(float& p, float g, float& m, float& v, const AdamCoef& c) {
+#pragma clang fp contract(off)
+    const float gg = __builtin_fmaf(g, c.gscale, c.wd * p);
+    const float gg2 = ((1.f - c.b2) * gg) * gg;
+    if (AMP) {
+        v = c.b2 * v + gg2;
+        m = __builtin_fmaf(1.f - c.b1, gg, c.b1 * m);
+    } else {
+        m = __builtin_fmaf(c.b1, m, (1.f - c.b1) * gg);
+        v = __builtin_fmaf(c.b2, v, gg2);
+    }
+    p = p - (c.step_size * m) / __builtin_fmaf(sqrtf(v), c.rsqrt_bc2, c.eps);
+}
+template <bool AMP>
+__device__ __forceinline__ f32x4 adam_update4(float* __restrict__ p, const float* __restrict__ g, float* __restrict__ m,
+                                              float* __restrict__ v, size_t i, const AdamCoef& c) {
+    f32x4 pv = *reinterpret_cast<f32x4*>(p + i);
+    const f32x4 gv = *reinterpret_cast<const f32x4*>(g + i);
+    f32x4 mv = *reinterpret_cast<f32x4*>(m + i), vv = *reinterpret_cast<f32x4*>(v + i);
+#pragma unroll
+    for (int e = 0; e < 4; ++e) {
+        float pe = pv[e], me = mv[e], ve = vv[e];
+        adam_update<AMP>(pe, gv[e], me, ve, c);
+        pv[e] = pe; mv[e] = me; vv[e] = ve;
+    }
+    *reinterpret_cast<f32x4*>(p + i) = pv;
+    *reinterpret_cast<f32x4*>(m + i) = mv;
+    *reinterpret_cast<f32x4*>(v + i) = vv;
+    return pv;
+}
+__device__ __forceinline__ AdamCoef adam_amp_coef(float lr, float b1, float b2, float eps, float wd, float gmul,
+                                                  const int* step, const float* loss_scale) {
+    const float t = (float)(step[0] + 1);
+    const float bc1 = 1.f - powf(b1, t), rsqrt_bc2 = rsqrtf(1.f - powf(b2, t));
+    const float gscale = gmul / (loss_scale ? loss_scale[0] : 1.f);
+    return AdamCoef{lr / bc1, b1, b2, eps, wd, rsqrt_bc2, gscale};
+}
 
 __global__ __launch_bounds__(256) void adam_kernel(float* __restrict__ p, const float* __restrict__ g,
                                                    float* __restrict__ m, float* __restrict__ v, size_t n, float lr,
                                                    float b1, float b2, float eps, float wd, float bc1, float rsqrt_bc2,
                                                    float gscale) {
+    const AdamCoef c{lr / bc1, b1, b2, eps, wd, rsqrt_bc2, gscale};
     const size_t stride = (size_t)gridDim.x * blockDim.x * 4;
     for (size_t i = ((size_t)blockIdx.x * blockDim.x + threadIdx.x) * 4; i < n; i += stride) {
         if (i + 3 < n) {
-            f32x4 pv = *reinterpret_cast<f32x4*>(p + i);
-            const f32x4 gv = *reinterpret_cast<const f32x4*>(g + i);
-            f32x4 mv = *reinterpret_cast<f32x4*>(m + i), vv = *reinterpret_cast<f32x4*>(v + i);
-#pragma unroll
-            for (int e = 0; e < 4; ++e) {
-                const float gg = gv[e] * gscale + wd * pv[e];
-                mv[e] = b1 * mv[e] + (1.f - b1) * gg;
-                vv[e] = b2 * vv[e] + (1.f - b2) * gg * gg;
-                pv[e] -= (lr / bc1) * mv[e] / (sqrtf(vv[e]) * rsqrt_bc2 + eps);
-            }
-            *reinterpret_cast<f32x4*>(p + i) = pv;
-            *reinterpret_cast<f32x4*>(m + i) = mv;
-            *reinterpret_cast<f32x4*>(v + i) = vv;
+            adam_update4<false>(p, g, m, v, i, c);
         } else {
-            for (size_t j = i; j < n; ++j) {
-                const float gg = g[j] * gscale + wd * p[j];
-                m[j] = b1 * m[j] + (1.f - b1) * gg;
-                v[j] = b2 * v[j] + (1.f - b2) * gg * gg;
-                p[j] -= (lr / bc1) * m[j] / (sqrtf(v[j]) * rsqrt_bc2 + eps);
-            }
+            for (size_t j = i; j < n; ++j) adam_update<false>(p[j], g[j], m[j], v[j], c);
         }
     }
 }
@@ -51,19 +75,11 @@
                                                        const int* __restrict__ step, const float* __restrict__ loss_scale,
                                                        const float* __restrict__ found_inf) {
     if (found_inf && found_inf[0] != 0.f) return;
-    const float t = (float)(step[0] + 1);
-    const float bc1 = 1.f - powf(b1, t), rsqrt_bc2 = rsqrtf(1.f - powf(b2, t));
-    const float gscale = gmul / (loss_scale ? loss_scale[0] : 1.f);
+    const AdamCoef c = adam_amp_coef(lr, b1, b2, eps, wd, gmul, step, loss_scale);
     const size_t stride = (size_t)gridDim.x * blockDim.x * 4;
     for (size_t i = ((size_t)blockIdx.x * blockDim.x + threadIdx.x) * 4; i < n; i += stride) {
         const size_t e1 = i + 4 < n ? i + 4 : n;
-        for (size_t j = i; j < e1; ++j) {
-            const float gg = g[j] * gscale + wd * p[j];
-            const float mj = b1 * m[j] + (1.f - b1) * gg, vj = b2 * v[j] + (1.f - b2) * gg * gg;
-            m[j] = mj;
-            v[j] = vj;
-            p[j] -= (lr / bc1) * mj / (sqrtf(vj) * rsqrt_bc2 + eps);
-        }
+        for (size_t j = i; j < e1; ++j) adam_update<true>(p[j], g[j], m[j], v[j], c);
     }
 }
 __global__ void adam_amp_advance_kernel(int* step, const float* found_inf) {
@@ -84,3 +100,179 @@
     MRISR_CHECK_LAUNCH("adam_step_amp(advance)");
     return MRISR_OK;
 }
+
+constexpr int kApTile = 32;
+constexpr int kApFlat = 1024;
+struct AdamPackSeg { long long off; int n, job0, njobs, tile0, ntiles, reserved_; };
+__host__ __device__ static inline int adam_pack_ext(int C) { return C >= 64 ? (C + 63) / 64 * 64 : (C + 31) / 32 * 32; }
+
+struct AdamPackArgs {
+    const PackJobDev* jobs;
+    const AdamPackSeg* segs;
+    int nsegs;
+    float *p, *m, *v;
+    const float* g;
+    size_t n;
+    float lr, b1, b2, eps, wd;
+    float bc1, rsqrt_bc2, gscale;
+    const int* step;
+    const float *loss_scale, *found_inf;
+};
+
+template <typename T, bool CHUNK_CO, typename F>
+__device__ __forceinline__ void adam_pack_emit(const float* tile, int ntaps, T* packed, F&& where) {
+    constexpr int EPC = 16 / (int)sizeof(T), KCH = kApTile / EPC;
+    const int nch = kApTile * ntaps * KCH;
+    for (int i = threadIdx.x; i < nch; i += blockDim.x) {
+        int row, kq, tap;
+        if (!CHUNK_CO) { kq = i % KCH; row = (i / KCH) % kApTile; tap = i / (KCH * kApTile); }
+        else { row = i % kApTile; kq = (i / kApTile) % KCH; tap = i / (kApTile * KCH); }
+        long long idx = where(row, tap, kq * EPC);
+        if (idx < 0) continue;
+        Vec16<T> v;
+#pragma unroll
+        for (int e = 0; e < EPC; ++e)
+            v.set(e, !CHUNK_CO ? tile[(row * ntaps + tap) * kApTile + kq * EPC + e] : tile[((kq * EPC + e) * ntaps + tap) * kApTile + row]);
+        store_vec16(packed + (size_t)idx * EPC, v);
+    }
+}
+
+template <typename T, bool AMP>
+__global__ __launch_bounds__(256) void adam_pack_kernel(const AdamPackArgs a) {
+    constexpr int EPC = 16 / (int)sizeof(T);
+    __shared__ float tile[kApTile * 9 * kApTile];
+    __shared__ int s_seg;
+    if (AMP && a.found_inf && a.found_inf[0] != 0.f) return;
+    const AdamCoef c = AMP ? adam_amp_coef(a.lr, a.b1, a.b2, a.eps, a.wd, a.gscale, a.step, a.loss_scale)
+                           : AdamCoef{a.lr / a.bc1, a.b1, a.b2, a.eps, a.wd, a.rsqrt_bc2, a.gscale};
+    const int b = blockIdx.x, t = threadIdx.x;
+    if (t == 0) s_seg = -1;
+    __syncthreads();
+    for (int i = t; i < a.nsegs; i += blockDim.x) {
+        const int t0 = a.segs[i].tile0;
+        if (b >= t0 && b < t0 + a.segs[i].ntiles) s_seg = i;
+    }
+    __syncthreads();
+    if (s_seg < 0) return;
+    const AdamPackSeg seg = a.segs[s_seg];
+    const int lt = b - seg.tile0;
+    float* __restrict__ p = a.p;
+    float* __restrict__ m = a.m;
+    float* __restrict__ v = a.v;
+    const float* __restrict__ g = a.g;
+    if (seg.njobs == 0) {
+        const size_t end = (size_t)seg.off + seg.n < a.n ? (size_t)seg.off + seg.n : a.n;
+        const size_t i = (size_t)seg.off + (size_t)lt * kApFlat + t * 4;
+        if (i + 3 < end) {
+            adam_update4<AMP>(p, g, m, v, i, c);
+        } else {
+            for (size_t j = i; j < end && j < i + 4; ++j) adam_update<AMP>(p[j], g[j], m[j], v[j], c);
+        }
+        return;
+    }
+    const PackJobDev j0 = a.jobs[seg.job0];
+    const int Cout = j0.Cout, Cin = j0.Cin, KS = j0.ksize, ntaps = KS * KS;
+    if (ntaps > 9 || (Cin & 3)) return;
+    const int ci_tiles = adam_pack_ext(Cin) / kApTile;
+    const int co0 = lt / ci_tiles * kApTile, ci0 = lt % ci_tiles * kApTile;
+    const int nvec = kApTile * ntaps * (kApTile / 4);
+#pragma unroll 3
+    for (int i = t; i < nvec; i += 256) {
+        const int c4 = i & 7, r = i >> 3, tap = r % ntaps, col = r / ntaps;
+        const int co = co0 + col, ci = ci0 + c4 * 4;
+        f32x4 pv = {0.f, 0.f, 0.f, 0.f};
+        const size_t idx = (size_t)seg.off + ((size_t)co * ntaps + tap) * Cin + ci;
+        if (co < Cout && ci < Cin && idx + 3 < a.n) pv = adam_update4<AMP>(p, g, m, v, idx, c);
+        *reinterpret_cast<f32x4*>(&tile[(col * ntaps + tap) * kApTile + c4 * 4]) = pv;
+    }
+    __syncthreads();
+    for (int jj = 0; jj < seg.njobs; ++jj) {
+        const PackJobDev j = a.jobs[seg.job0 + jj];
+        const int flip = j.flip & 1;
+        const int Co = flip ? Cin : Cout, Ci = flip ? Cout : Cin;
+        T* packed = (T*)j.packed;
+        if (j.flip & MRISR_PACK_UPADJ) {
+            if (!conv_upadj_image_bytes(TypeTraits<T>::kDtype, Cout, Cin, KS)) continue;
+            const PackUpadj L(Cout, ntaps);
+            adam_pack_emit<T, true>(tile, ntaps, packed, [&](int row, int tap, int kq) -> long long {
+                const int ci = ci0 + row, co = co0 + kq;
+                return ci < Cin && co < Cout ? (long long)L.encode(ci, L.row_of(co, tap), EPC) : -1;
+            });
+            if (co0 == 0) {
+                const int npad = (L.RS - L.K9) / EPC;
+                Vec16<T> z;
+                z.zero();
+                for (int i = t; i < kApTile * npad; i += 256) {
+                    const int ci = ci0 + i % kApTile;
+                    if (ci < Cin) store_vec16(packed + L.encode(ci, L.K9 + i / kApTile * EPC, EPC) * EPC, z);
+                }
+            }
+        } else if (j.flip & MRISR_PACK_RING) {
+            const PackRing L(TypeTraits<T>::kDtype, Co, Ci, KS);
+            if (L.RBN == 0) continue;
+            auto where = [&](int mco, int mtap, int mci) -> long long {
+                int co, tap, k;
+                pack_image_coord(flip, ntaps, mco, mtap, mci, co, tap, k);
+                return co < L.rows() && k < L.chans() ? (long long)L.encode(co, tap, k) : -1;
+            };
+            if (!flip) adam_pack_emit<T, false>(tile, ntaps, packed, [&](int row, int tap, int kq) { return where(co0 + row, tap, ci0 + kq); });
+            else adam_pack_emit<T, true>(tile, ntaps, packed, [&](int row, int tap, int kq) { return where(co0 + kq, tap, ci0 + row); });
+        } else {
+            const PackPlain<T> L(Co, Ci, ntaps);
+            auto where = [&](int mco, int mtap, int mci) -> long long {
+                int co, tap, k;
+                pack_image_coord(flip, ntaps, mco, mtap, mci, co, tap, k);
+                return co < L.rows() && k < L.chans() ? (long long)L.encode(co, tap, k) : -1;
+            };
+            if (!flip) adam_pack_emit<T, false>(tile, ntaps, packed, [&](int row, int tap, int kq) { return where(co0 + row, tap, ci0 + kq); });
+            else adam_pack_emit<T, true>(tile, ntaps, packed, [&](int row, int tap, int kq) { return where(co0 + kq, tap, ci0 + row); });
+        }
+    }
+}
+
+extern "C" int mrisr_adam_pack_tiles(int Cout, int Cin, int ksize) {
+    if (Cout < 1 || Cin < 1 || (Cin & 3) || (ksize != 1 && ksize != 3)) return 0;
+    return (adam_pack_ext(Cout) / kApTile) * (adam_pack_ext(Cin) / kApTile);
+}
+extern "C" int mrisr_adam_pack_flat_tile(void) { return kApFlat; }
+
+template <bool AMP>
+static int adam_pack_launch(const char* name, int dtype, const AdamPackArgs& a, int ntiles, void* stream) {
+    static_assert(sizeof(AdamPackSeg) == sizeof(mrisr_adam_pack_seg), "mrisr_adam_pack_seg layout");
+    static_assert(sizeof(PackJobDev) == sizeof(mrisr_pack_job), "mrisr_pack_job layout");
+    if (!a.p || !a.g || !a.m || !a.v || !a.jobs || !a.segs) MRISR_FAIL(MRISR_E_ARG, "%s: null pointer", name);
+    if (((uintptr_t)a.p | (uintptr_t)a.g | (uintptr_t)a.m | (uintptr_t)a.v) & 15) MRISR_FAIL(MRISR_E_ARG, "%s: buffers must be 16-byte aligned", name);
+    if (a.nsegs < 1 || ntiles < 1) MRISR_FAIL(MRISR_E_ARG, "%s: empty segment table", name);
+    if (dtype == MRISR_BF16) adam_pack_kernel<bf16_t, AMP><<<ntiles, 256, 0, (hipStream_t)stream>>>(a);
+    else if (dtype == MRISR_F16) adam_pack_kernel<f16_t, AMP><<<ntiles, 256, 0, (hipStream_t)stream>>>(a);
+    else if (dtype == MRISR_F32) adam_pack_kernel<float, AMP><<<ntiles, 256, 0, (hipStream_t)stream>>>(a);
+    else MRISR_FAIL(MRISR_E_DTYPE, "%s: dtype %d", name, dtype);
+    MRISR_CHECK_LAUNCH(name);
+    return MRISR_OK;
+}
+
+extern "C" int mrisr_adam_pack_step(int dtype, float* p, const float* g, float* m, float* v, size_t n, float lr, float beta1,
+                                    float beta2, float eps, float weight_decay, int step, float grad_scale,
+                                    const mrisr_pack_job* jobs_device, const mrisr_adam_pack_seg* segs_device, int nsegs,
+                                    int ntiles, void* stream) {
+    if (step < 1) MRISR_FAIL(MRISR_E_ARG, "adam_pack_step: step %d < 1", step);
+    const double bc1 = 1.0 - pow((double)beta1, step), bc2 = 1.0 - pow((double)beta2, step);
+    const AdamPackArgs a{(const PackJobDev*)jobs_device, (const AdamPackSeg*)segs_device, nsegs, p, m, v, g, n, lr, beta1, beta2,
+                         eps, weight_decay, (float)bc1, (float)(1.0 / sqrt(bc2)), grad_scale, nullptr, nullptr, nullptr};
+    return adam_pack_launch<false>("adam_pack_step", dtype, a, ntiles, stream);
+}
+
+extern "C" int mrisr_adam_pack_step_amp(int dtype, float* p, const float* g, float* m, float* v, size_t n, float lr,
+                                        float beta1, float beta2, float eps, float weight_decay, int* step_device,
+                                        float grad_mul, const float* loss_scale_device, const float* found_inf_device,
+                                        const mrisr_pack_job* jobs_device, const mrisr_adam_pack_seg* segs_device, int nsegs,
+                                        int ntiles, void* stream) {
+    if (!step_device) MRISR_FAIL(MRISR_E_ARG, "adam_pack_step_amp: null pointer");
+    const AdamPackArgs a{(const PackJobDev*)jobs_device, (const AdamPackSeg*)segs_device, nsegs, p, m, v, g, n, lr, beta1, beta2,
+                         eps, weight_decay, 1.f, 1.f, grad_mul, step_device, loss_scale_device, found_inf_device};
+    const int rc = adam_pack_launch<true>("adam_pack_step_amp", dtype, a, ntiles, stream);
+    if (rc != MRISR_OK) return rc;
+    adam_amp_advance_kernel<<<1, 1, 0, (hipStream_t)stream>>>(step_device, found_inf_device);
+    MRISR_CHECK_LAUNCH("adam_pack_step_amp(advance)");
+    return MRISR_OK;
+}
diff --git a/mri_superresolution_amd/engine.py b/mri_superresolution_amd/engine.py
--- a/mri_superresolution_amd/engine.py
+++ b/mri_superresolution_amd/engine.py
@@ -199,40 +199,97 @@
         self._packed.clear()
         self._jobs_key = None
         self._packed_token = None
-
-    def _pack_all(self, params, dt: int, stream, token=None):
+        self._adam_table = None
+
+    def _build_jobs(self, params, dt: int):
         dev = params[self.layers[0].name + ".weight"].device
         key = (dt, str(dev), tuple(params[l.name + ".weight"].data_ptr() for l in self.layers))
-        if getattr(self, "_jobs_key", None) != key:
-            jobs = (L.PackJob * (4 * len(self.layers) + 1))()
-            i = 0
-            for layer in self.layers:
-                w = params[layer.name + ".weight"]
-                for flip in (0, 1):
-                    buf = self._packed_buf(layer, w, dt, flip)
-                    j = jobs[i]
-                    j.w, j.packed, j.Cout, j.Cin, j.ksize, j.transpose_flip = w.data_ptr(), buf.data_ptr(), layer.cout, layer.cin, layer.ks, flip
-                    i += 1
-                    co, ci = (layer.cin, layer.cout) if flip else (layer.cout, layer.cin)
-                    if L.load().mrisr_conv_ring_bn(dt, co, ci, layer.ks) > 0:
-                        buf = self._packed_buf(layer, w, dt, flip, ring=True)
-                        j = jobs[i]
-                        j.w, j.packed, j.Cout, j.Cin, j.ksize, j.transpose_flip = (w.data_ptr(), buf.data_ptr(), layer.cout, layer.cin,
-                                                                                   layer.ks, flip | L.PACK_RING)
-                        i += 1
-                if layer.up_src and L.load().mrisr_packed_weight_bytes_upadj(dt, layer.cout, layer.cin, layer.ks) > 0:
-                    buf = self._packed_buf(layer, w, dt, 0, upadj=True)
+        if getattr(self, "_jobs_key", None) == key:
+            return
+        jobs = (L.PackJob * (4 * len(self.layers) + 1))()
+        ranges = {}
+        i = 0
+        for layer in self.layers:
+            w = params[layer.name + ".weight"]
+            first = i
+            for flip in (0, 1):
+                buf = self._packed_buf(layer, w, dt, flip)
+                j = jobs[i]
+                j.w, j.packed, j.Cout, j.Cin, j.ksize, j.transpose_flip = w.data_ptr(), buf.data_ptr(), layer.cout, layer.cin, layer.ks, flip
+                i += 1
+                co, ci = (layer.cin, layer.cout) if flip else (layer.cout, layer.cin)
+                if L.load().mrisr_conv_ring_bn(dt, co, ci, layer.ks) > 0:
+                    buf = self._packed_buf(layer, w, dt, flip, ring=True)
                     j = jobs[i]
                     j.w, j.packed, j.Cout, j.Cin, j.ksize, j.transpose_flip = (w.data_ptr(), buf.data_ptr(), layer.cout, layer.cin,
-                                                                               layer.ks, L.PACK_UPADJ)
+                                                                               layer.ks, flip | L.PACK_RING)
                     i += 1
-            self._jobs_bytes = sum(4 * params[l.name + ".weight"].numel() for l in self.layers) * 2 + \
-                sum(b.numel() for k, b in self._packed.items() if k[1] == dt)
-            host = torch.frombuffer(bytearray(bytes(jobs)), dtype=torch.uint8)
-            self._jobs_dev = host.to(dev)
-            self._jobs_n = i
-            self._jobs_key = key
+            if layer.up_src and L.load().mrisr_packed_weight_bytes_upadj(dt, layer.cout, layer.cin, layer.ks) > 0:
+                buf = self._packed_buf(layer, w, dt, 0, upadj=True)
+                j = jobs[i]
+                j.w, j.packed, j.Cout, j.Cin, j.ksize, j.transpose_flip = (w.data_ptr(), buf.data_ptr(), layer.cout, layer.cin,
+                                                                           layer.ks, L.PACK_UPADJ)
+                i += 1
+            ranges[layer.name] = (first, i - first)
+        self._jobs_bytes = sum(4 * params[l.name + ".weight"].numel() for l in self.layers) * 2 + \
+            sum(b.numel() for k, b in self._packed.items() if k[1] == dt)
+        host = torch.frombuffer(bytearray(bytes(jobs)), dtype=torch.uint8)
+        self._jobs_dev = host.to(dev)
+        self._jobs_n = i
+        self._jobs_key = key
+        self._job_ranges = ranges
+        self._adam_table = None
+
+    def _pack_all(self, params, dt: int, stream, token=None):
+        self._build_jobs(params, dt)
         L.call("mrisr_pack_weights_batched", dt, self._jobs_dev.data_ptr(), self._jobs_n, stream, nbytes=self._jobs_bytes)
+        self._packed_token = (dt, token)
+
+    def adam_pack_table(self, params, flat: torch.Tensor, offsets):
+        if self._packed_token is None or getattr(self, "_jobs_key", None) is None:
+            return None
+        dt = self._packed_token[0]
+        key = (dt, str(flat.device), tuple(params[l.name + ".weight"].data_ptr() for l in self.layers))
+        if key != self._jobs_key:
+            return None
+        if self._adam_table is None:
+            lib = L.load()
+            ftile = lib.mrisr_adam_pack_flat_tile()
+            segs, pos, tile = [], 0, 0
+            base, n = flat.data_ptr(), flat.numel()
+
+            def plain(lo, hi):
+                nonlocal tile
+                if hi > lo:
+                    nt = -(-(hi - lo) // ftile)
+                    segs.append((lo, hi - lo, 0, 0, tile, nt))
+                    tile += nt
+            for layer in sorted(self.layers, key=lambda l: offsets[l.name + ".weight"][0]):
+                off, cnt = offsets[layer.name + ".weight"]
+                nt = lib.mrisr_adam_pack_tiles(layer.cout, layer.cin, layer.ks)
+                if nt <= 0 or off % 4 or params[layer.name + ".weight"].data_ptr() != base + 4 * off or off < pos:
+                    self._adam_table = False
+                    return None
+                plain(pos, off)
+                j0, nj = self._job_ranges[layer.name]
+                segs.append((off, cnt, j0, nj, tile, nt))
+                tile += nt
+                pos = off + cnt
+            plain(pos, n)
+            arr = (L.AdamPackSeg * len(segs))()
+            for a, (off, cnt, j0, nj, t0, nt) in zip(arr, segs):
+                a.off, a.n, a.job0, a.njobs, a.tile0, a.ntiles = off, cnt, j0, nj, t0, nt
+            dev = torch.frombuffer(bytearray(bytes(arr)), dtype=torch.uint8).to(flat.device)
+            self._adam_table = (dev, len(segs), tile, sum(b.numel() for k, b in self._packed.items() if k[1] == dt))
+        if self._adam_table is False:
+            return None
+        dev, nsegs, ntiles, img_bytes = self._adam_table
+        return dt, self._jobs_dev.data_ptr(), dev.data_ptr(), nsegs, ntiles, img_bytes
+
+    def images_current(self, dt: int, token) -> bool:
+        return token is not None and self._packed_token == (dt, token)
+
+    def images_written(self, dt: int, token):
         self._packed_token = (dt, token)
 
     def _desc(self, layer: Layer, p: _Pass, dt: int, params, fused_blend: bool = False) -> L.ConvDesc:
@@ -294,7 +351,7 @@
             o = ns[n]
             o.scale, o.shift, o.meanrstd = gn_finalize(o.stats, params[n.gamma], params[n.beta], N, n.C, o.H, o.W, st)
 
-        if training or weights_token is None or self._packed_token != (dt, weights_token):
+        if not self.images_current(dt, weights_token):
             self._pack_all(params, dt, st, weights_token)
         s = ns[self.stem]
         s.H, s.W = H, W
diff --git a/mri_superresolution_amd/optim.py b/mri_superresolution_amd/optim.py
--- a/mri_superresolution_amd/optim.py
+++ b/mri_superresolution_amd/optim.py
@@ -17,6 +17,7 @@
         self._step_dev = None
         self.device_step = bool(device_step)
         self.dp_grad_scale = 1.0
+        self.fuse_pack = True
         self._alloc()
 
     def _alloc(self):
@@ -41,23 +42,30 @@
             if p.grad is not None and p.grad.data_ptr() != gv.data_ptr():
                 gv.copy_(p.grad)
         g = self.param_groups[0]
+        fused = m._engine.adam_pack_table(m._param_dict(), m.flat_params, m._offsets) if self.fuse_pack else None
+        n = m.flat_params.numel()
+        bufs = (m.flat_params.data_ptr(), m.flat_grads.data_ptr(), self.exp_avg.data_ptr(), self.exp_avg_sq.data_ptr(), n)
+        hyper = (float(g["lr"]), float(g["betas"][0]), float(g["betas"][1]), float(g["eps"]), float(g["weight_decay"]))
+        if fused is not None:
+            dt, jobs, segs, nsegs, ntiles, img_bytes = fused
+            pre, post, suffix, nbytes = (dt,), (jobs, segs, nsegs, ntiles), "_pack", 28 * n + img_bytes
+        else:
+            pre, post, suffix, nbytes = (), (), "", 28 * n
         loss_scale, found_inf = getattr(self, "grad_scale", None), getattr(self, "found_inf", None)
         if loss_scale is not None or found_inf is not None or self._step_dev is not None or self.device_step:
             if self._step_dev is None:
                 self._step_dev = torch.tensor([self._step], dtype=torch.int32, device=m.flat_params.device)
             ls = None if loss_scale is None else loss_scale.detach().to(torch.float32).reshape(-1)
             fi = None if found_inf is None else found_inf.detach().to(torch.float32).reshape(-1)
-            L.call("mrisr_adam_step_amp", m.flat_params.data_ptr(), m.flat_grads.data_ptr(), self.exp_avg.data_ptr(),
-                   self.exp_avg_sq.data_ptr(), m.flat_params.numel(), float(g["lr"]), float(g["betas"][0]),
-                   float(g["betas"][1]), float(g["eps"]), float(g["weight_decay"]), self._step_dev.data_ptr(),
-                   float(self.dp_grad_scale), L.ptr(ls), L.ptr(fi), L.stream_ptr(), nbytes=28 * m.flat_params.numel())
+            L.call(f"mrisr_adam{suffix}_step_amp", *pre, *bufs, *hyper, self._step_dev.data_ptr(), float(self.dp_grad_scale),
+                   L.ptr(ls), L.ptr(fi), *post, L.stream_ptr(), nbytes=nbytes)
         else:
             self._step += 1
-            L.call("mrisr_adam_step", m.flat_params.data_ptr(), m.flat_grads.data_ptr(), self.exp_avg.data_ptr(),
-                   self.exp_avg_sq.data_ptr(), m.flat_params.numel(), float(g["lr"]), float(g["betas"][0]),
-                   float(g["betas"][1]), float(g["eps"]), float(g["weight_decay"]), self._step, float(self.dp_grad_scale),
-                   L.stream_ptr(), nbytes=28 * m.flat_params.numel())
+            L.call(f"mrisr_adam{suffix}_step", *pre, *bufs, *hyper, self._step, float(self.dp_grad_scale), *post,
+                   L.stream_ptr(), nbytes=nbytes)
         m.mark_weights_changed()
+        if fused is not None:
+            m._engine.images_written(fused[0], m._weights_token())
         return loss
 
     def _views(self, flat):
```

Result: no change. 2188 slices/s (median of 2 runs) (+0.0%).
